# huangnengCSU/longcallR

Hardware: AMD Instinct MI355X
Metric: candidate_sites_per_sec (higher is better)
Workload: dtype u8 in, u32 counts, f64 likelihoods, i64 fixed-point phase scores

## Files before the change

longcallr_amd/csrc/k2_candidates.hip:

```cpp
#include "lcr_dev.h"
#include "k2_eval.h"

#define SCAN_ITEMS 4
#define SCAN_TILE (LCR_BLOCK * SCAN_ITEMS)

__device__ __forceinline__ int wave_incl_scan_i(int v, int lane) {
#pragma unroll
  for (int d = 1; d < 64; d <<= 1) {
    int t = __shfl_up(v, d, 64);
    if (lane >= d) v += t;
  }
  return v;
}
__device__ __forceinline__ long long wave_incl_scan_ll(long long v, int lane) {
#pragma unroll
  for (int d = 1; d < 64; d <<= 1) {
    long long t = __shfl_up(v, d, 64);
    if (lane >= d) v += t;
  }
  return v;
}

template <typename OutT>
__global__ void __launch_bounds__(LCR_BLOCK) scan_phase1(const int32_t* __restrict__ in, OutT* __restrict__ out, int32_t n,
                                                         long long* __restrict__ block_sum) {
  __shared__ long long wsum[4];
  const int tid = threadIdx.x, lane = tid & 63, w = tid >> 6;
  const long long base = (long long)blockIdx.x * SCAN_TILE + (long long)tid * SCAN_ITEMS;
  long long v[SCAN_ITEMS], s = 0;
#pragma unroll
  for (int k = 0; k < SCAN_ITEMS; k++) { v[k] = (base + k < n) ? (long long)in[base + k] : 0; s += v[k]; }
  long long incl = wave_incl_scan_ll(s, lane);
  if (lane == 63) wsum[w] = incl;
  __syncthreads();
  long long add = 0;
  for (int i = 0; i < w; i++) add += wsum[i];
  long long run = incl - s + add;
#pragma unroll
  for (int k = 0; k < SCAN_ITEMS; k++) { if (base + k < n) out[base + k] = (OutT)run; run += v[k]; }
  if (tid == LCR_BLOCK - 1) block_sum[blockIdx.x] = incl + add;
}
__global__ void __launch_bounds__(1024) scan_phase2(long long* __restrict__ block_sum, int32_t n_blocks, long long* total) {
  __shared__ long long wsum[16];
  __shared__ long long carry_s;
  const int tid = threadIdx.x, lane = tid & 63, w = tid >> 6;
  if (tid == 0) carry_s = 0;
  __syncthreads();
  for (int base = 0; base < n_blocks; base += 1024) {
    long long v = (base + tid < n_blocks) ? block_sum[base + tid] : 0;
    long long incl = wave_incl_scan_ll(v, lane);
    if (lane == 63) wsum[w] = incl;
    __syncthreads();
    long long add = carry_s;
    for (int i = 0; i < w; i++) add += wsum[i];
    if (base + tid < n_blocks) block_sum[base + tid] = incl - v + add;
    __syncthreads();
    if (tid == 1023) carry_s = incl + add;
    __syncthreads();
  }
  if (tid == 0 && total) *total = carry_s;
}
template <typename OutT>
__global__ void __launch_bounds__(LCR_BLOCK) scan_phase3(OutT* __restrict__ out, int32_t n, const long long* __restrict__ block_sum,
                                                         int write_last) {
  const long long base = (long long)blockIdx.x * SCAN_TILE + (long long)threadIdx.x * SCAN_ITEMS;
  const long long add = block_sum[blockIdx.x];
#pragma unroll
  for (int k = 0; k < SCAN_ITEMS; k++) if (base + k < n) out[base + k] += (OutT)add;
  (void)write_last;
}
#define SCAN_FUSED_BLOCKS 2048
template <typename OutT>
__global__ void __launch_bounds__(LCR_BLOCK) scan_phase3x(OutT* __restrict__ out, int32_t n, const long long* __restrict__ block_sum, int32_t n_blocks,
                                                          int32_t* __restrict__ total32, int64_t* __restrict__ total64) {
  __shared__ long long wsum[LCR_BLOCK / 64];
  const int tid = threadIdx.x, lane = tid & 63, w = tid >> 6;
  long long s = 0;
  for (int j = tid; j < (int)blockIdx.x; j += LCR_BLOCK) s += block_sum[j];
  for (int d = 32; d >= 1; d >>= 1) s += __shfl_xor(s, d, 64);
  if (lane == 0) wsum[w] = s;
  __syncthreads();
  long long add = 0;
#pragma unroll
  for (int i = 0; i < LCR_BLOCK / 64; i++) add += wsum[i];
  const long long base = (long long)blockIdx.x * SCAN_TILE + (long long)tid * SCAN_ITEMS;
#pragma unroll
  for (int k = 0; k < SCAN_ITEMS; k++) if (base + k < n) out[base + k] += (OutT)add;
  if ((int)blockIdx.x == n_blocks - 1 && tid == 0) {
    const long long tot = add + block_sum[n_blocks - 1];
    if (total32) *total32 = (int32_t)tot;
    if (total64) *total64 = (int64_t)tot;
  }
}
__global__ void write_total_i32(const long long* total, int32_t* dst) { *dst = (int32_t)*total; }
__global__ void gather_i32(const int32_t* __restrict__ src, const int32_t* __restrict__ idx, int32_t n, int32_t n_src,
                           const int32_t* __restrict__ total, int32_t* __restrict__ out, int32_t* __restrict__ host_out) {
  const int i = blockIdx.x * blockDim.x + threadIdx.x;
  if (i < n) { const int32_t v = idx[i] < n_src ? src[idx[i]] : *total; out[i] = v; if (host_out) host_out[i] = v; }
}
void launch_gather_i32(const int32_t* src, const int32_t* idx, int32_t n, int32_t n_src, const int32_t* total, int32_t* out, hipStream_t s, int32_t* host_out) {
  if (n > 0) hipLaunchKernelGGL(gather_i32, dim3((n + 255) / 256), dim3(256), 0, s, src, idx, n, n_src, total, out, host_out);
}
__global__ void write_total_i64(const long long* total, int64_t* dst) { *dst = (int64_t)*total; }

void launch_scan_i32(DevBuf& tmp, const int32_t* in, int32_t* out_excl, int32_t n, int32_t* total, hipStream_t s) {
  const int nb = (n + SCAN_TILE - 1) / SCAN_TILE;
  (void)tmp.reserve(((size_t)nb + 2) * sizeof(long long));
  long long* bs = tmp.as<long long>();
  if (n > 0 && nb <= SCAN_FUSED_BLOCKS) {
    hipLaunchKernelGGL(scan_phase1<int32_t>, dim3(nb), dim3(LCR_BLOCK), 0, s, in, out_excl, n, bs);
    hipLaunchKernelGGL(scan_phase3x<int32_t>, dim3(nb), dim3(LCR_BLOCK), 0, s, out_excl, n, bs, nb, total, (int64_t*)nullptr);
  } else if (n > 0) {
    hipLaunchKernelGGL(scan_phase1<int32_t>, dim3(nb), dim3(LCR_BLOCK), 0, s, in, out_excl, n, bs);
    hipLaunchKernelGGL(scan_phase2, dim3(1), dim3(1024), 0, s, bs, nb, bs + nb);
    hipLaunchKernelGGL(scan_phase3<int32_t>, dim3(nb), dim3(LCR_BLOCK), 0, s, out_excl, n, bs, 0);
    if (total) hipLaunchKernelGGL(write_total_i32, dim3(1), dim3(1), 0, s, bs + nb, total);
  } else if (total) {
    (void)hipMemsetAsync(total, 0, sizeof(int32_t), s);
  }
}
void launch_scan_i32_to_i64(DevBuf& tmp, const int32_t* in, int64_t* out_excl, int32_t n, hipStream_t s) {
  const int nb = (n + SCAN_TILE - 1) / SCAN_TILE;
  (void)tmp.reserve(((size_t)nb + 2) * sizeof(long long));
  long long* bs = tmp.as<long long>();
  if (n > 0 && nb <= SCAN_FUSED_BLOCKS) {
    hipLaunchKernelGGL(scan_phase1<int64_t>, dim3(nb), dim3(LCR_BLOCK), 0, s, in, out_excl, n, bs);
    hipLaunchKernelGGL(scan_phase3x<int64_t>, dim3(nb), dim3(LCR_BLOCK), 0, s, out_excl, n, bs, nb, (int32_t*)nullptr, out_excl + n);
  } else if (n > 0) {
    hipLaunchKernelGGL(scan_phase1<int64_t>, dim3(nb), dim3(LCR_BLOCK), 0, s, in, out_excl, n, bs);
    hipLaunchKernelGGL(scan_phase2, dim3(1), dim3(1024), 0, s, bs, nb, bs + nb);
    hipLaunchKernelGGL(scan_phase3<int64_t>, dim3(nb), dim3(LCR_BLOCK), 0, s, out_excl, n, bs, 0);
    hipLaunchKernelGGL(write_total_i64, dim3(1), dim3(1), 0, s, bs + nb, out_excl + n);
  } else {
    (void)hipMemsetAsync(out_excl, 0, sizeof(int64_t), s);
  }
}

__global__ void k2_sor_threshold(float* out) { *out = strand_odds_ratio(5, 5, 9, 1); }

__device__ __forceinline__ ColEval eval_column(const uint32_t* __restrict__ planes, int64_t n_cols, int64_t o, uint8_t ref_base,
                                               const DevParams& prm, const BinomTable& bt) {
  uint32_t cnt[4];
#pragma unroll
  for (int k = 0; k < 4; k++) { cnt[k] = planes[(int64_t)(LCR_PL_A + k) * n_cols + o]; }
  return eval_counts(cnt, ref_base, prm, bt,
                     [&]() { return planes[(int64_t)LCR_PL_D * n_cols + o]; }, [&]() { return planes[(int64_t)LCR_PL_N * n_cols + o]; },
                     [&](int k) { return planes[(int64_t)(LCR_PL_FWD_A + k) * n_cols + o]; });
}

__global__ void __launch_bounds__(LCR_BLOCK)
k2_filter(BatchView b, DevParams prm, BinomTable bt, const int32_t* __restrict__ tile_region, const int32_t* __restrict__ tile_col0,
          int64_t n_cols, const uint32_t* __restrict__ planes, const int32_t* __restrict__ tile_fill, uint8_t* __restrict__ flags,
          int32_t* __restrict__ tile_count) {
  __shared__ int cnt_s;
  if (tile_fill[blockIdx.x] == 0) { if (threadIdx.x == 0) tile_count[blockIdx.x] = 0; return; }
  const int g = tile_region[blockIdx.x], tc0 = tile_col0[blockIdx.x];
  const int tlen = min(LCR_TILE, b.len[g] - tc0);
  const int64_t gcol0 = b.col_off[g] + tc0;
  if (threadIdx.x == 0) cnt_s = 0;
  __syncthreads();
  int mine = 0;
  for (int col = threadIdx.x; col < tlen; col += LCR_BLOCK) {
    ColEval ev = eval_column(planes, n_cols, gcol0 + col, b.ref[gcol0 + col], prm, bt);
    flags[gcol0 + col] = ev.pass ? 1 : 0;
    mine += ev.pass ? 1 : 0;
  }
  if (mine) atomicAdd(&cnt_s, mine);
  __syncthreads();
  if (threadIdx.x == 0) tile_count[blockIdx.x] = cnt_s;
}

void launch_k2_filter(const BatchView& b, const DevParams& p, const int32_t* tile_region, const int32_t* tile_col0,
                      int32_t n_tiles, int64_t n_cols, const uint32_t* planes, const int32_t* tile_fill, uint8_t* flags,
                      int32_t* tile_count, hipStream_t s) {
  static const BinomTable bt = make_binom_table();
  if (n_tiles == 0) return;
  hipLaunchKernelGGL(k2_filter, dim3(n_tiles), dim3(LCR_BLOCK), 0, s, b, p, bt, tile_region, tile_col0, n_cols, planes,
                     tile_fill, flags, tile_count);
}

__global__ void __launch_bounds__(LCR_BLOCK)
k2_compact(BatchView b, DevParams prm, BinomTable bt, const int32_t* __restrict__ tile_region,
           const int32_t* __restrict__ tile_col0, int64_t n_cols, const uint32_t* __restrict__ planes,
           const uint8_t* __restrict__ flags, const int32_t* __restrict__ tile_count, const int32_t* __restrict__ tile_off,
           Survivor* __restrict__ out, int32_t out_cap ) {
  __shared__ int wsum[4];
  if (tile_count[blockIdx.x] == 0) return;
  const int g = tile_region[blockIdx.x], tc0 = tile_col0[blockIdx.x];
  const int tlen = min(LCR_TILE, b.len[g] - tc0);
  const int64_t gcol0 = b.col_off[g] + tc0;
  const int tid = threadIdx.x, lane = tid & 63, w = tid >> 6;
  int base = tile_off[blockIdx.x];
  int f[4], c = 0;
#pragma unroll
  for (int k = 0; k < 4; k++) { int col = tid * 4 + k; f[k] = (col < tlen) ? flags[gcol0 + col] : 0; c += f[k]; }
  int incl = wave_incl_scan_i(c, lane);
  if (lane == 63) wsum[w] = incl;
  __syncthreads();
  int add = 0;
  for (int i = 0; i < w; i++) add += wsum[i];
  int rank = base + incl - c + add;
#pragma unroll
  for (int k = 0; k < 4; k++) {
    if (!f[k]) continue;
    const int col = tid * 4 + k;
    ColEval ev = eval_column(planes, n_cols, gcol0 + col, b.ref[gcol0 + col], prm, bt);
    Survivor sv;
    sv.gcol = gcol0 + col; sv.region = g; sv.col = tc0 + col;
    sv.ref_base = ev.ref_base; sv.allele1 = ev.allele1; sv.allele2 = ev.allele2; sv.n_alt = ev.n_alt;
    sv.cnt1 = ev.cnt1; sv.cnt2 = ev.cnt2; sv.depth = ev.depth; sv.af1 = ev.af1; sv.af2 = ev.af2;
    sv.ts_fwd = planes[(int64_t)LCR_PL_TS_FWD * n_cols + gcol0 + col];
    sv.ts_rev = planes[(int64_t)LCR_PL_TS_REV * n_cols + gcol0 + col];
    if (rank < out_cap) out[rank] = sv;
    rank++;
  }
}


__global__ void __launch_bounds__(LCR_BLOCK)
k2_hist(BatchView b, DevParams prm, const ReadBin* __restrict__ rbin, const Survivor* __restrict__ sv,
        const int32_t* __restrict__ tile_off, int32_t n_tiles, int32_t n_sv, uint32_t* __restrict__ hist, int32_t* __restrict__ hit_cnt, uint2* __restrict__ hit_list,
        int32_t* __restrict__ ovf_cnt, int32_t* __restrict__ ovf_list) {
  const int r = (blockIdx.x * LCR_BLOCK + threadIdx.x) >> 4;
  const bool live = r < b.n_reads;
  const int rr = live ? r : 0;
  const ReadBin h = rbin[rr];
  const int rend = b.read_rend[rr];
  const uint8_t* __restrict__ seq = b.bases + h.seq_off;
  const uint8_t* __restrict__ qual = b.quals + h.seq_off;
  const int l16 = threadIdx.x & 15, rbase = threadIdx.x & 48;
  const int key = h.rel_pos > 0 ? h.rel_pos : 0, rend_c = min(rend, h.vec);
  const bool span = live && rend_c > key;
  const int t0 = h.ftile + (int)((unsigned int)key / (unsigned int)LCR_TILE), t1 = h.ftile + (int)((unsigned int)(max(rend_c, 1) - 1) / (unsigned int)LCR_TILE) + 1;
  uint32_t pre[4];
  {
    const uint32_t* __restrict__ cg = b.cigar + h.cig_off;
#pragma unroll
    for (int k = 0; k < 4; k++) pre[k] = (span && (uint32_t)(16 * k + l16) < (uint32_t)h.n_cig) ? cg[16 * k + l16] : 0u;
  }
  const int s_lo = span ? tile_off[t0] : 0, s_hi = span ? (t1 < n_tiles ? tile_off[t1] : n_sv) : 0;
  int nh = 0;
  uint2* const hl = hit_cnt ? hit_list + (size_t)rr * LCR_HITS : nullptr;
  int cur, s_end;
  auto site_col = [&](int i) { return sv[i].col; };
  row16_find_sites(span && s_lo < s_hi, h, rend, s_lo, s_hi, site_col, &cur, &s_end);
  row16_walk_range(b, h, cur, s_end, pre, site_col,
    [&](int cur_s, int c, bool hit) {
      uint8_t base = 0, rq = 0;
      if (hit) { base = seq[c]; rq = qual[c]; }
      if (hl) {
        const unsigned int hm = (unsigned int)(__ballot(hit) >> rbase) & 0xffffu;
        const int at = nh + __popc(hm & ((1u << l16) - 1u));
        if (hit && at < LCR_HITS) hl[at] = make_uint2((uint32_t)cur_s, (uint32_t)base | ((uint32_t)rq << 8));
        nh += __popc(hm);
      }
      if (!hit) return;
      const uint8_t bq = rq < 30 ? rq : 30;
      bool masked = false;
      if (in_end_zone(c, h.lead, h.reb, prm.dist_to_end))
        masked = prm.ont ? true : polya_masked(seq, b.seq_len[rr], c, prm.polya_len, sv[cur_s].ref_base);
      const int bi = base_code(base);
      if (!masked && bi >= 0) atomicAdd(&hist[((int64_t)cur_s * 4 + bi) * 31 + bq], 1u);
    });
  if (hl && live && l16 == 0) {
    hit_cnt[r] = nh;
    if (nh > LCR_HITS) ovf_list[atomicAdd(ovf_cnt, 1)] = r;
  }
}

void launch_k2_hist(const BatchView& b, const DevParams& p, const ReadBin* rbin, const Survivor* sv,
                    const int32_t* tile_off, int32_t n_tiles, int32_t n_sv, uint32_t* hist, int32_t* hit_cnt, void* hit_list, int32_t* ovf_cnt, int32_t* ovf_list, hipStream_t s) {
  if (b.n_reads == 0) return;
  const int per = LCR_BLOCK / 16;
  hipLaunchKernelGGL(k2_hist, dim3((b.n_reads + per - 1) / per), dim3(LCR_BLOCK), 0, s, b, p, rbin, sv, tile_off, n_tiles, n_sv, hist, hit_cnt, (uint2*)hit_list,
                     ovf_cnt, ovf_list);
}

#ifndef HT_SLOTS
#define HT_SLOTS 256
#endif
#ifndef HT_SPLIT
#define HT_SPLIT 32
#endif
#ifndef HT_BLOCK
#define HT_BLOCK 512
#endif
__global__ void __launch_bounds__(HT_BLOCK)
k2_hist_tiles(BatchView b, const int32_t* __restrict__ tile_col0, const int32_t* __restrict__ tile_count, const int32_t* __restrict__ tile_off,
              const Survivor* __restrict__ sv, const int32_t* __restrict__ ent_off, const uint2* __restrict__ ents,
              const unsigned long long* __restrict__ recs, uint32_t* __restrict__ hist) {
  const int tile = blockIdx.x / HT_SPLIT, part = blockIdx.x % HT_SPLIT, cnt = tile_count[tile];
  if (cnt == 0) return;
  __shared__ uint32_t hp[HT_SLOTS * 62];
  __shared__ uint16_t slot_of[LCR_TILE];
  constexpr int HT_LANES = 8;
  const int tid = threadIdx.x, grp = tid / HT_LANES, ln = tid % HT_LANES;
  const int s0 = tile_off[tile], tc0 = tile_col0[tile];
  const int e0 = ent_off[tile];
  const int n_ent = ent_off[tile + 1] - e0;
  const int j_lo = 16 * (int)((int64_t)n_ent * part / HT_SPLIT), j_hi = 16 * (int)((int64_t)n_ent * (part + 1) / HT_SPLIT);
  if (j_lo >= j_hi) return;
  for (int p0 = 0; p0 < cnt; p0 += HT_SLOTS) {
    const int pc = min(HT_SLOTS, cnt - p0);
    for (int i = tid; i < LCR_TILE; i += HT_BLOCK) slot_of[i] = 0xFFFFu;
    for (int i = tid; i < pc * 62; i += HT_BLOCK) hp[i] = 0u;
    __syncthreads();
    for (int i = tid; i < pc; i += HT_BLOCK) slot_of[sv[s0 + p0 + i].col - tc0] = (uint16_t)i;
    __syncthreads();
    const int c_lo = sv[s0 + p0].col - tc0, c_hi = sv[s0 + p0 + pc - 1].col - tc0;
    auto fetch = [&](int j) -> unsigned long long {
      if (j >= j_hi) return ~0ull;
      const uint2 en = ents[e0 + (j >> 4)];
      return ((unsigned int)j & 15u) < en.y ? recs[en.x + ((unsigned int)j & 15u)] : ~0ull;
    };
    unsigned long long nx = fetch(j_lo + grp), nx2 = fetch(j_lo + grp + HT_BLOCK / HT_LANES);
    for (int j = j_lo + grp; j < j_hi; j += HT_BLOCK / HT_LANES) {
      const unsigned long long rec = nx;
      nx = nx2;
      nx2 = fetch(j + 2 * (HT_BLOCK / HT_LANES));
      const unsigned long long off = rec & REC_OFF_MASK;
      const bool live = off < REC_KIND_N;
      const int col0 = (int)((rec >> 40) & 1023u), len = (int)((rec >> 50) & 1023u) + 1;
      const int d_lo = max(0, c_lo - col0), d_hi = live ? min(len - 1, c_hi - col0) : -1;
      auto tally = [&](int dd, bool in, uint32_t base, uint32_t qual) {
        const uint32_t slot = slot_of[min(col0 + max(dd, 0), LCR_TILE - 1)];
        const uint32_t u = (base & 0xDFu) - 65u;
        const bool acgt = u < 20u && ((0x80045u >> u) & 1u);
        const uint32_t k = ((base & 0xDFu) >> 1) & 3u, bi = k ^ (k >> 1);
        const uint32_t q = min(qual, 30u);
        const uint32_t idx = slot * 124u + bi * 31u + q;
        if (in && acgt && slot != 0xFFFFu) atomicAdd(&hp[idx >> 1], 1u << (16 * (idx & 1u)));
      };
      for (int d0 = d_lo + 4 * ln; d0 <= d_hi; d0 += 4 * HT_LANES) {
        const unsigned long long at = off + (unsigned long long)d0;
        uint32_t bw, qw;
        if (at + 4 <= (unsigned long long)b.n_bases) {
          bw = *reinterpret_cast<const uint32_t*>(b.bases + at); qw = *reinterpret_cast<const uint32_t*>(b.quals + at);
        } else {
          bw = 0; qw = 0;
          for (int t = 0; t < 4; t++) if (at + t < (unsigned long long)b.n_bases) { bw |= (uint32_t)b.bases[at + t] << (8 * t); qw |= (uint32_t)b.quals[at + t] << (8 * t); }
        }
#pragma unroll
        for (int t = 0; t < 4; t++) tally(d0 + t, d0 + t <= d_hi, (bw >> (8 * t)) & 0xFFu, (qw >> (8 * t)) & 0xFFu);
      }
    }
    __syncthreads();
    uint32_t* out = hist + (int64_t)(s0 + p0) * 124;
    for (int i = tid; i < pc * 124; i += HT_BLOCK) {
      const uint32_t v = (hp[i >> 1] >> (16 * (i & 1))) & 0xffffu;
      if (v) atomicAdd(&out[i], v);
    }
    __syncthreads();
  }
}

void launch_k2_hist_tiles(const BatchView& b, const int32_t* tile_col0, int32_t n_tiles, const int32_t* tile_count,
                          const int32_t* tile_off, const Survivor* sv, const int32_t* ent_off, const void* ents, const unsigned long long* recs,
                          uint32_t* hist , hipStream_t s) {
  if (n_tiles == 0) return;
  hipLaunchKernelGGL(k2_hist_tiles, dim3((unsigned)n_tiles * HT_SPLIT), dim3(HT_BLOCK), 0, s, b, tile_col0, tile_count, tile_off, sv, ent_off,
                     (const uint2*)ents, recs, hist);
}

struct GtConst {
  double le[31], l1e[31];
  double log10_2;
  double log_prior[3];
};
static GtConst make_gt_const() {
  GtConst c;
  for (int q = 0; q <= 30; q++) {
    double e = pow(0.1, (double)q / 10.0);
    c.le[q] = log10(e);
    c.l1e[q] = log10(1.0 - e);
  }
  c.log10_2 = log10(2.0);
  const double theta = 0.001;
  c.log_prior[0] = log10(theta / 2.0); c.log_prior[1] = log10(theta); c.log_prior[2] = log10(1.0 - 1.5 * theta);
  return c;
}

__global__ void __launch_bounds__(LCR_BLOCK)
k2_gt(DevParams prm, GtConst gc, const Survivor* __restrict__ sv, int32_t n_sv, const uint32_t* __restrict__ hist,
      const int64_t* __restrict__ start0, lcr_candidate* __restrict__ out, int32_t* __restrict__ keep) {
  const int s = blockIdx.x * blockDim.x + threadIdx.x;
  if (s >= n_sv) return;
  const Survivor v = sv[s];
  const uint32_t* h = hist + (int64_t)s * 124;
  keep[s] = 0;
  const int ri = base_code(v.ref_base);
  {
    int ai = -1; uint32_t ac = 0;
    if (v.allele1 != v.ref_base) { ai = base_code(v.allele1); ac = v.cnt1; }
    else if (v.allele2 != v.ref_base) { ai = base_code(v.allele2); ac = v.cnt2; }
    if (ai >= 0) {
      uint32_t pass = 0;
      for (uint32_t q = prm.min_baseq; q <= 30; q++) pass += h[ai * 31 + q];
      if (ac > 0 && pass < 2) return;
    }
  }
  double l0 = 0.0, l2 = 0.0;
  uint32_t num_reads = 0;
  for (int q = 0; q <= 30; q++) {
    const uint32_t hm = h[ri * 31 + q];
    uint32_t hx = 0;
#pragma unroll
    for (int bq = 0; bq < 4; bq++) if (bq != ri) hx += h[bq * 31 + q];
    num_reads += hm + hx;
    if (hm) { l0 += (double)hm * gc.le[q]; l2 += (double)hm * gc.l1e[q]; }
    if (hx) { l0 += (double)hx * gc.l1e[q]; l2 += (double)hx * gc.le[q]; }
  }
  double loglik[3] = {l0, 0.0, l2};
  loglik[1] -= (double)num_reads * gc.log10_2;
  double logprob[3] = {loglik[0] + gc.log_prior[0], loglik[1] + gc.log_prior[1], loglik[2] + gc.log_prior[2]};
  const double mlp = fmax(fmax(logprob[0], logprob[1]), logprob[2]);
  double vp[3] = {pow(10.0, logprob[0] - mlp), pow(10.0, logprob[1] - mlp), pow(10.0, logprob[2] - mlp)};
  const double svp = vp[0] + vp[1] + vp[2];
  vp[2] = vp[2] / svp;
  const double variant_quality = -10.0 * log10(fmax(10e-301, vp[2]));
  const double ml = fmax(fmax(loglik[0], loglik[1]), loglik[2]);
  double gl[3] = {pow(10.0, loglik[0] - ml), pow(10.0, loglik[1] - ml), pow(10.0, loglik[2] - ml)};
  const double sgl = gl[0] + gl[1] + gl[2];
  double gp[3] = {gl[0] / sgl, gl[1] / sgl, gl[2] / sgl};
  double ph[3] = {-10.0 * log10(gp[0]), -10.0 * log10(gp[1]), -10.0 * log10(gp[2])};
  for (int i = 1; i < 3; i++) {
    double x = ph[i];
    int j = i;
    while (j > 0 && x < ph[j - 1]) { ph[j] = ph[j - 1]; j--; }
    ph[j] = x;
  }
  const double genotype_quality = ph[1] - ph[0];

  lcr_candidate c;
  c.pos = start0[v.region] + v.col;
  c.region = v.region;
  c.ref_base = v.ref_base; c.allele1 = v.allele1; c.allele2 = v.allele2; c.n_alt = v.n_alt;
  c.cnt1 = v.cnt1; c.cnt2 = v.cnt2; c.depth = v.depth; c.af1 = v.af1; c.af2 = v.af2;
  c.haplotype = 0; c.phase_set = 0; c.phase_score = 0.0;
  for (int k = 0; k < 3; k++) { c.loglik[k] = loglik[k]; c.gt_prob[k] = gp[k]; }
  c.qual = variant_quality; c.gq = genotype_quality;
  if (gp[0] > gp[1] && gp[0] > gp[2]) { c.variant_type = 2; c.genotype = -1; }
  else if (gp[1] > gp[0] && gp[1] > gp[2]) { c.variant_type = 1; c.genotype = 0; }
  else { c.variant_type = 0; c.genotype = 1; }
  c.flags = 0;
  if (variant_quality < (double)prm.min_qual) return;
  uint8_t ref_allele_base, alt0; float altf0, altf1 = 0.0f;
  if (v.allele1 == v.ref_base) { ref_allele_base = v.allele1; alt0 = v.allele2; altf0 = v.af2; }
  else if (v.allele2 == v.ref_base) { ref_allele_base = v.allele2; alt0 = v.allele1; altf0 = v.af1; }
  else { ref_allele_base = v.ref_base; alt0 = v.allele1; altf0 = v.af1; altf1 = v.af2; }
  const int fwd_t = (int)v.ts_fwd, rev_t = (int)v.ts_rev;
  bool kept = false;
  if (ref_allele_base == 'A' && alt0 == 'G' && (fwd_t > rev_t * 2 || (fwd_t == 0 && rev_t == 0)) && c.variant_type != 2) {
    c.flags = LCR_F_RNA_EDIT; kept = true;
  } else if (ref_allele_base == 'T' && alt0 == 'C' && (rev_t > fwd_t * 2 || (fwd_t == 0 && rev_t == 0)) && c.variant_type != 2) {
    c.flags = LCR_F_RNA_EDIT; kept = true;
  } else if (v.n_alt == 1 && altf0 < prm.min_af) {
    c.flags = LCR_F_CAND_SOMATIC; kept = true;
  } else if (c.variant_type == 2) {
    if (v.n_alt == 2 && altf0 >= prm.min_af && altf1 >= prm.min_af) { c.variant_type = 3; c.genotype = -1; }
    c.flags = LCR_F_HOM | LCR_F_FOR_PHASING; kept = true;
  } else if (c.variant_type == 1) {
    if (v.n_alt == 2) { c.variant_type = 3; c.genotype = -1; c.flags = LCR_F_HOM | LCR_F_FOR_PHASING; }
    else c.flags = LCR_F_HET | LCR_F_FOR_PHASING;
    kept = true;
  }
  if (!kept) return;
  out[s] = c;
  keep[s] = 1;
}

void launch_k2_gt(const DevParams& p, const Survivor* sv, int32_t n_sv, const uint32_t* hist, const int64_t* start0,
                  lcr_candidate* out, int32_t* keep, hipStream_t s) {
  static const GtConst g_gtc = make_gt_const();
  if (n_sv == 0) return;
  hipLaunchKernelGGL(k2_gt, dim3((n_sv + LCR_BLOCK - 1) / LCR_BLOCK), dim3(LCR_BLOCK), 0, s, p, g_gtc, sv, n_sv, hist, start0, out, keep);
}

void launch_k2_compact(const BatchView& b, const DevParams& p, const int32_t* tile_region, const int32_t* tile_col0,
                       int32_t n_tiles, int64_t n_cols, const uint32_t* planes, const uint8_t* flags,
                       const int32_t* tile_count, const int32_t* tile_off, Survivor* out, int32_t out_cap, hipStream_t s) {
  static const BinomTable bt = make_binom_table();
  if (n_tiles == 0) return;
  hipLaunchKernelGGL(k2_compact, dim3(n_tiles), dim3(LCR_BLOCK), 0, s, b, p, bt, tile_region, tile_col0, n_cols,
                     planes, flags, tile_count, tile_off, out, out_cap);
}

float lcr_device_sor_threshold(hipStream_t s) {
  float* d = nullptr;
  float h = 0.f;
  if (hipMalloc(&d, sizeof(float)) != hipSuccess) return 0.f;
  hipLaunchKernelGGL(k2_sor_threshold, dim3(1), dim3(1), 0, s, d);
  (void)hipMemcpyAsync(&h, d, sizeof(float), hipMemcpyDeviceToHost, s);
  (void)hipStreamSynchronize(s);
  (void)hipFree(d);
  return h;
}

__global__ void __launch_bounds__(LCR_BLOCK)
k2_scatter(const lcr_candidate* __restrict__ tmp, const int32_t* __restrict__ keep, const int32_t* __restrict__ pos, int32_t n_sv,
           lcr_candidate* __restrict__ out, const int32_t* __restrict__ sv_region_off, int32_t n_regions, int32_t* __restrict__ cand_off) {
  const int64_t id = (int64_t)blockIdx.x * LCR_BLOCK + threadIdx.x;
  if (id <= n_regions) cand_off[id] = sv_region_off[id] < n_sv ? pos[sv_region_off[id]] : pos[n_sv];
  const int s = (int)(id >> 3), w = (int)(id & 7);
  if (s >= n_sv || !keep[s]) return;
  reinterpret_cast<uint4*>(out + pos[s])[w] = reinterpret_cast<const uint4*>(tmp + s)[w];
}
__global__ void __launch_bounds__(256)
k2_dense(lcr_candidate* __restrict__ cand, const int32_t* __restrict__ cand_off, int32_t n_regions, int32_t* __restrict__ idx,
         uint32_t dense_win, uint32_t min_dense_cnt, lcr_candidate* __restrict__ h_cand, int32_t* __restrict__ h_off) {
  __shared__ int wcnt[4], base_s;
  const int g = blockIdx.x, tid = threadIdx.x, lane = tid & 63, w = tid >> 6;
  const int lo = cand_off[g], hi = cand_off[g + 1];
  int32_t* concat = idx + lo;
  if (tid == 0) base_s = 0;
  __syncthreads();
  for (int i0 = lo; i0 < hi; i0 += 256) {
    const int i = i0 + tid;
    const bool keep = i < hi && (cand[i].flags & (LCR_F_HOM | LCR_F_HET)) != 0;
    const unsigned long long m = __ballot(keep);
    if (lane == 0) wcnt[w] = __popcll(m);
    __syncthreads();
    int before = base_s;
    for (int k = 0; k < w; k++) before += wcnt[k];
    if (keep) concat[before + __popcll(m & ((1ull << lane) - 1ull))] = i;
    __syncthreads();
    if (tid == 0) base_s += wcnt[0] + wcnt[1] + wcnt[2] + wcnt[3];
    __syncthreads();
  }
  const int n = base_s;
  auto mark = [&](int i, int j) {
    for (int tk = i; tk < j; tk++) { atomicOr(&cand[concat[tk]].flags, (uint32_t)LCR_F_DENSE); atomicAnd(&cand[concat[tk]].flags, ~(uint32_t)LCR_F_FOR_PHASING); }
  };
  auto sweep = [&](int i, int64_t W, uint32_t cnt) {
    const int64_t start_pos = cand[concat[i]].pos;
    int j = i;
    while (j < n && cand[concat[j]].pos - start_pos <= W) j++;
    if (j < n) { if ((uint32_t)(j - i) >= cnt) mark(i, j); }
    else if ((uint32_t)(n - i) >= cnt) mark(i, n - 1);
  };
  for (int i = tid; i < n; i += 256) {
    sweep(i, (int64_t)dense_win, min_dense_cnt);
    sweep(i, 4, 3u);
  }
  if (!h_cand) return;
  __syncthreads();
  const uint4* src = reinterpret_cast<const uint4*>(cand + lo);
  uint4* dst = reinterpret_cast<uint4*>(h_cand + lo);
  const int n16 = (hi - lo) * (int)(sizeof(lcr_candidate) / 16);
  for (int i = tid; i < n16; i += 256) dst[i] = src[i];
  if (tid == 0) { h_off[g] = lo; if (g == n_regions - 1) h_off[n_regions] = hi; }
}
void launch_k2_finish(DevBuf& scan_tmp, const lcr_candidate* tmp, const int32_t* keep, int32_t n_sv, const int32_t* sv_region_off,
                      int32_t n_regions, int32_t* pos , int32_t* idx , lcr_candidate* out,
                      int32_t* cand_off , uint32_t dense_win, uint32_t min_dense_cnt, hipStream_t s,
                      lcr_candidate* h_cand , int32_t* h_off ) {
  static_assert(sizeof(lcr_candidate) % 16 == 0, "k2_dense exports 16-byte words");
  launch_scan_i32(scan_tmp, keep, pos, n_sv, pos + n_sv, s);
  if (n_sv > 0) {
    const int64_t nthreads = std::max<int64_t>((int64_t)n_sv * 8, (int64_t)n_regions + 1);
    hipLaunchKernelGGL(k2_scatter, dim3((unsigned)((nthreads + LCR_BLOCK - 1) / LCR_BLOCK)), dim3(LCR_BLOCK), 0, s, tmp, keep, pos, n_sv, out,
                       sv_region_off, n_regions, cand_off);
  } else launch_gather_i32(pos, sv_region_off, n_regions + 1, n_sv, pos + n_sv, cand_off, s);
  if (n_regions > 0) hipLaunchKernelGGL(k2_dense, dim3(n_regions), dim3(256), 0, s, out, cand_off, n_regions, idx, dense_win, min_dense_cnt, h_cand, h_off);
}
```

longcallr_amd/csrc/lcr_api.hip:

```cpp
#include <atomic>
#include <thread>
#include <algorithm>
#include <cmath>
#include <cstring>
#include <cstdlib>

#include <chrono>
#include "lcr_dev.h"
#include "lcr_phase_host.h"

struct lcr_ctx {
  int device = 0;
  hipStream_t stream = nullptr;
  bool own_stream = false;
  std::string err;

  bool loaded = false;
  BatchView bv{};
  int64_t n_cols = 0, n_bases = 0, n_cigar = 0;
  int32_t n_tiles = 0;
  std::vector<int64_t> h_start0, h_col_off;
  std::vector<int32_t> h_len, h_read_begin, h_region_first_tile;
  DevBuf in_[16];
  struct UploadSlot { DevBuf buf[16]; hipEvent_t ev = nullptr; bool filled = false; lcr_reads rd{}; lcr_regions rg{}; } up[2];
  hipStream_t up_stream = nullptr;
  hipEvent_t ev_dl = nullptr, ev_cand_dl = nullptr;
  bool cand_dl_other = false;
  int bound_slot = -1;
  bool bound_host = false;
  DevBuf scan_tmp, read_region, read_bin, read_rend, tile_region, tile_col0, first_tile, k0_tile_fill, k0_items, tile_nbase, tile_order;
  DevBuf desc_tile, desc_val, chunks, chunk_off;
  DevBuf blk_first_read, read_scan, cig_compact, cig_off_new, cig_new_off32;
  uint64_t cig0 = 0;
  uint32_t n_ops = 0;
  int64_t n_items = 0;

  bool have_planes = false;
  DevBuf planes;
  DevParams dp{};
  int32_t pile_platform = -1; uint32_t pile_dist_to_end = 0;
  float sor_thr = -1.f;
  HostBuf h_planes;
  HostBuf h_nnz;
  DevBuf region_e_off, frag_tmp_col, frag_tmp_val;
  hipEvent_t ev_nnz = nullptr, ev_cand = nullptr, ev_ctl = nullptr, ev_sv = nullptr;
  int32_t sv_cap_guess = 0;
  bool nnz_pending = false, cand_pending = false;
  HostBuf h_order;
  static constexpr int UP_LANES = 4;
  HostBuf h_up[2 * UP_LANES]; hipEvent_t ev_up[2 * UP_LANES] = {}; bool up_busy[2 * UP_LANES] = {};
  HostBuf h_stage[4];

  bool have_cand = false;
  bool cand_used = false;
  DevBuf flags, tile_count, tile_off, total, survivors, sv_region_off, hist, cand_tmp, keep;
  DevBuf hit_cnt, hit_list, ovf_list;
  bool hits_valid = false; int32_t hits_n_sv = 0;
  int dbg_hist_tiles = 0;
  int dbg_spec_compact = 1;
  int dbg_fuse_filter = 1;
  bool flt_fused = false;
  DevParams flt_dp{};
  int dbg_k3_hits = 1;
  std::vector<lcr_candidate> h_cand;
  std::vector<int32_t> h_cand_off;
  DevBuf d_cand, d_cand_off;
  DevBuf imp_pos, imp_gt, imp_q, imp_cnt;
  HostBuf h_imp_bad;
  hipEvent_t ev_imp = nullptr;

  bool have_frag = false;
  uint32_t min_linkers = 1;
  int32_t n_rows = 0;
  int64_t nnz = 0;
  std::vector<int32_t> h_row_region_off;
  DevBuf region_rows, row_region_off, row_cnt, row_links, row_ptr, col, val;
  HostBuf h_row_ptr, h_row_read, h_col, h_val, h_row_fp, h_row_links;

  bool have_phase = false;
  bool res_valid = false;
  int32_t res_ng = 0;
  int phase_slot = -1;
  PhaseHost phase;
  std::vector<int32_t> ld_off, ld_snps;

  DevBuf rd_start, rd_end, rd_diff, rd_ex, rd_cnt, rd_off, rd_s, rd_e, rd_max;
  std::vector<int64_t> rl_start0;
  std::vector<int32_t> rl_len;
  std::vector<uint32_t> rl_max;

  bool timing = false;
  uint32_t timing_mask = 0;
  hipEvent_t ev[LCR_NKERNELS][2] = {};
  bool ev_valid[LCR_NKERNELS] = {};
  int64_t pileup_bytes = 0, stage_bytes = 0;
};

#include <map>
#include <mutex>
namespace {
struct BlockCache {
  std::mutex mu;
  std::multimap<size_t, void*> blocks[2][16];
  size_t held[2][16] = {};
  size_t limit[2] = {(size_t)24 << 30, (size_t)2 << 30};
};
BlockCache& block_cache() { static BlockCache* c = new BlockCache(); return *c; }
}
void* lcr_cache_take(int host, size_t want, size_t* cap) {
  int dev = 0;
  if (hipGetDevice(&dev) != hipSuccess || dev < 0 || dev >= 16) return nullptr;
  BlockCache& bc = block_cache();
  std::lock_guard<std::mutex> g(bc.mu);
  auto& m = bc.blocks[host ? 1 : 0][dev];
  auto it = m.lower_bound(want);
  if (it == m.end() || it->first > 2 * want + (1u << 20)) return nullptr;
  void* p = it->second;
  *cap = it->first;
  bc.held[host ? 1 : 0][dev] -= it->first;
  m.erase(it);
  return p;
}
bool lcr_cache_put(int host, void* p, size_t cap) {
  int dev = 0;
  if (!p || hipGetDevice(&dev) != hipSuccess || dev < 0 || dev >= 16) return false;
  BlockCache& bc = block_cache();
  std::lock_guard<std::mutex> g(bc.mu);
  const int h = host ? 1 : 0;
  if (bc.held[h][dev] + cap > bc.limit[h]) return false;
  bc.blocks[h][dev].emplace(cap, p);
  bc.held[h][dev] += cap;
  return true;
}

namespace {

struct Timer {
  lcr_ctx* c; int k;
  bool on() const { return c->timing && (c->timing_mask == 0 || ((c->timing_mask >> k) & 1u)); }
  Timer(lcr_ctx* c_, int k_) : c(c_), k(k_) { if (on()) { (void)hipEventRecord(c->ev[k][0], c->stream); } }
  ~Timer() { if (on()) { (void)hipEventRecord(c->ev[k][1], c->stream); c->ev_valid[k] = true; } }
};

DevParams to_dev(const lcr_params* p, float sor_thr) {
  DevParams d{};
  d.ont = p->platform == LCR_PLATFORM_ONT;
  d.dist_to_end = (int32_t)p->dist_to_end;
  d.polya_len = (int32_t)p->polya_len;
  d.min_baseq = p->min_baseq; d.min_depth = p->min_depth; d.max_depth = p->max_depth; d.min_qual = p->min_qual;
  d.low_cnt_cut = p->low_cnt_cut; d.min_linkers = p->min_linkers; d.use_strand_bias = p->use_strand_bias;
  d.min_af = p->min_af; d.min_af_intron = p->min_af_intron; d.low_frac_cut = p->low_frac_cut;
  d.sor_threshold = sor_thr;
  return d;
}

int upload_bytes(lcr_ctx* c, void* dst, const void* src, size_t bytes, hipStream_t q = nullptr) {
  if (!q) q = c->stream;
  if (bytes <= 64 * 1024) { HIPCHK(c, hipMemcpyAsync(dst, src, bytes, hipMemcpyHostToDevice, q)); return LCR_OK; }
  hipPointerAttribute_t at{};
  if (hipPointerGetAttributes(&at, src) == hipSuccess && at.type == hipMemoryTypeHost) {
    HIPCHK(c, hipMemcpyAsync(dst, src, bytes, hipMemcpyHostToDevice, q));
    return LCR_OK;
  }
  (void)hipGetLastError();
  constexpr size_t CH = 8u << 20;
  const int lanes = bytes >= (64u << 20) ? lcr_ctx::UP_LANES : 1;
  for (int k = 0; k < 2 * lanes; k++) {
    HIPCHK(c, c->h_up[k].reserve(CH));
    if (!c->ev_up[k]) HIPCHK(c, hipEventCreateWithFlags(&c->ev_up[k], hipEventDisableTiming));
  }
  const size_t n_ch = (bytes + CH - 1) / CH;
  std::atomic<int> bad{0};
  auto lane_fn = [&](int w) {
    (void)hipSetDevice(c->device);
    int use = 0;
    for (size_t i = (size_t)w; i < n_ch && !bad.load(std::memory_order_relaxed); i += (size_t)lanes, use ^= 1) {
      const int k = 2 * w + use;
      const size_t off = i * CH, n = std::min(CH, bytes - off);
      hipError_t e = c->up_busy[k] ? hipEventSynchronize(c->ev_up[k]) : hipSuccess;
      if (e == hipSuccess) {
        memcpy(c->h_up[k].p, (const uint8_t*)src + off, n);
        e = hipMemcpyAsync((uint8_t*)dst + off, c->h_up[k].p, n, hipMemcpyHostToDevice, q);
      }
      if (e == hipSuccess) e = hipEventRecord(c->ev_up[k], q);
      if (e != hipSuccess) { bad.store((int)e); return; }
      c->up_busy[k] = true;
    }
  };
  if (lanes == 1) lane_fn(0);
  else {
    std::vector<std::thread> th;
    try { for (int w = 1; w < lanes; w++) th.emplace_back(lane_fn, w); } catch (...) { }
    const int started = (int)th.size() + 1;
    lane_fn(0);
    for (auto& t : th) t.join();
    for (int w = started; w < lanes; w++) lane_fn(w);
  }
  if (bad.load()) { c->err = std::string("host upload: ") + hipGetErrorString((hipError_t)bad.load()); return LCR_E_DEVICE; }
  return LCR_OK;
}

template <class T>
int upload(lcr_ctx* c, DevBuf& buf, const T* src, size_t n, const T** dst, int mem) {
  if (mem == LCR_MEM_DEVICE) { *dst = src; return LCR_OK; }
  HIPCHK(c, buf.reserve(std::max<size_t>(n, 1) * sizeof(T)));
  if (n) { const int rc = upload_bytes(c, buf.p, src, n * sizeof(T)); if (rc) return rc; }
  *dst = buf.as<T>();
  return LCR_OK;
}

}

int g_lcr_own_fill = 1;
namespace {
__global__ void __launch_bounds__(256) lcr_fill_kernel(uint8_t* p, uint32_t word, size_t head, size_t n16, size_t tail) {
  const size_t t = (size_t)blockIdx.x * blockDim.x + threadIdx.x, nt = (size_t)gridDim.x * blockDim.x;
  if (t < head) p[t] = (uint8_t)word;
  uint4* const body = reinterpret_cast<uint4*>(p + head);
  const uint4 w = make_uint4(word, word, word, word);
  for (size_t i = t; i < n16; i += nt) body[i] = w;
  if (t < tail) p[head + 16 * n16 + t] = (uint8_t)word;
}
}
namespace {
struct FillRanges { uint8_t* p[4]; size_t head[4], n16[4], tail[4]; uint32_t word[4]; };
__global__ void __launch_bounds__(256) lcr_fill_multi_kernel(FillRanges r) {
  const int k = blockIdx.y;
  uint8_t* const p = r.p[k];
  if (!p) return;
  const size_t t = (size_t)blockIdx.x * blockDim.x + threadIdx.x, nt = (size_t)gridDim.x * blockDim.x;
  const uint32_t word = r.word[k];
  if (t < r.head[k]) p[t] = (uint8_t)word;
  uint4* const body = reinterpret_cast<uint4*>(p + r.head[k]);
  const uint4 w = make_uint4(word, word, word, word);
  for (size_t i = t; i < r.n16[k]; i += nt) body[i] = w;
  if (t < r.tail[k]) p[r.head[k] + 16 * r.n16[k] + t] = (uint8_t)word;
}
}
hipError_t lcr_fill_multi_async(int n, void* const* ptrs, const int* bytes_val, const size_t* sizes, hipStream_t s) {
  if (!g_lcr_own_fill) { for (int k = 0; k < n; k++) if (sizes[k]) { const hipError_t e = hipMemsetAsync(ptrs[k], bytes_val[k], sizes[k], s); if (e != hipSuccess) return e; } return hipSuccess; }
  FillRanges r{};
  size_t most = 0;
  int m = 0;
  for (int k = 0; k < n && m < 4; k++) {
    if (!sizes[k]) continue;
    const size_t mis = (size_t)((uintptr_t)ptrs[k] & 15), head = std::min(sizes[k], mis ? 16 - mis : 0), n16 = (sizes[k] - head) / 16;
    const uint32_t b = (uint32_t)(bytes_val[k] & 255);
    r.p[m] = (uint8_t*)ptrs[k]; r.head[m] = head; r.n16[m] = n16; r.tail[m] = sizes[k] - head - 16 * n16; r.word[m] = b | (b << 8) | (b << 16) | (b << 24);
    most = std::max(most, n16); m++;
  }
  if (!m) return hipSuccess;
  const unsigned blocks = (unsigned)std::max<size_t>(1, std::min<size_t>((most + 255) / 256, 1024));
  hipLaunchKernelGGL(lcr_fill_multi_kernel, dim3(blocks, (unsigned)m), dim3(256), 0, s, r);
  return hipGetLastError();
}

hipError_t lcr_fill_async(void* p, int byte, size_t bytes, hipStream_t s) {
  if (!bytes) return hipSuccess;
  if (!g_lcr_own_fill) return hipMemsetAsync(p, byte, bytes, s);
  const size_t mis = (size_t)((uintptr_t)p & 15), head = std::min(bytes, mis ? 16 - mis : 0), n16 = (bytes - head) / 16, tail = bytes - head - 16 * n16;
  const uint32_t b = (uint32_t)(byte & 255), word = b | (b << 8) | (b << 16) | (b << 24);
  const unsigned blocks = (unsigned)std::max<size_t>(1, std::min<size_t>((n16 + 255) / 256, 2048));
  hipLaunchKernelGGL(lcr_fill_kernel, dim3(blocks), dim3(256), 0, s, (uint8_t*)p, word, head, n16, tail);
  return hipGetLastError();
}

int g_lcr_host_trace = 0;
namespace {
struct HtMark { const char* tag; std::chrono::steady_clock::time_point t; };
thread_local std::vector<HtMark> g_ht;
}
void lcr_host_trace_mark(const char* tag) { g_ht.push_back({tag, std::chrono::steady_clock::now()}); }
void lcr_host_trace_flush() {
  if (g_ht.empty()) return;
  std::string line = "[host]";
  char buf[96];
  for (const HtMark& m : g_ht) { snprintf(buf, sizeof buf, " %s %.1f", m.tag, std::chrono::duration<double, std::micro>(m.t - g_ht[0].t).count()); line += buf; }
  fprintf(stderr, "%s\n", line.c_str());
  g_ht.clear();
}

extern "C" {

const char* lcr_version(void) { return "liblcr 0.1 (gfx950)"; }

int lcr_release_cached_memory(void) {
  BlockCache& bc = block_cache();
  std::lock_guard<std::mutex> g(bc.mu);
  int cur = 0;
  (void)hipGetDevice(&cur);
  for (int dev = 0; dev < 16; dev++) {
    if (bc.blocks[0][dev].empty() && bc.blocks[1][dev].empty()) continue;
    (void)hipSetDevice(dev);
    for (auto& kv : bc.blocks[0][dev]) (void)hipFree(kv.second);
    for (auto& kv : bc.blocks[1][dev]) (void)hipHostFree(kv.second);
    bc.blocks[0][dev].clear(); bc.blocks[1][dev].clear();
    bc.held[0][dev] = bc.held[1][dev] = 0;
  }
  (void)hipSetDevice(cur);
  return LCR_OK;
}
int lcr_set_cache_limits(int64_t device_bytes, int64_t host_bytes) {
  if (device_bytes < 0 || host_bytes < 0) return LCR_E_ARG;
  BlockCache& bc = block_cache();
  std::lock_guard<std::mutex> g(bc.mu);
  bc.limit[0] = (size_t)device_bytes; bc.limit[1] = (size_t)host_bytes;
  return LCR_OK;
}

int lcr_params_preset(int preset, lcr_params* o) {
  if (!o || preset < 0 || preset > 3) return LCR_E_ARG;
  memset(o, 0, sizeof *o);
  const bool ont = preset >= 2;
  o->platform = ont ? LCR_PLATFORM_ONT : LCR_PLATFORM_HIFI;
  o->min_baseq = 10; o->dist_to_end = ont ? 20 : 40; o->polya_len = 5;
  o->min_depth = ont ? 10 : 6; o->max_depth = 50000; o->min_qual = 2;
  o->dense_win = 100; o->min_dense_cnt = 5; o->low_cnt_cut = 10; o->min_linkers = 1; o->max_enum_snps = 10;
  o->ld_weight_threshold = 1;
  o->use_strand_bias = (preset == 0 || preset == 2) ? 1 : 0;
  o->min_af = ont ? 0.20f : 0.15f; o->min_af_intron = 0.0f; o->low_frac_cut = 0.05f;
  o->min_phase_score = ont ? 13.0f : 11.0f;
  o->read_assign_cutoff = 0.0; o->seed = 2025;
  return LCR_OK;
}

int lcr_ctx_create(int device, lcr_ctx** out) {
  if (!out) return LCR_E_ARG;
  int n = 0;
  if (hipGetDeviceCount(&n) != hipSuccess || n <= 0 || device < 0 || device >= n) return LCR_E_DEVICE;
  if (hipSetDevice(device) != hipSuccess) return LCR_E_DEVICE;
  lcr_ctx* c = new lcr_ctx();
  c->device = device;
  if (hipStreamCreateWithFlags(&c->stream, hipStreamNonBlocking) != hipSuccess) { delete c; return LCR_E_DEVICE; }
  c->own_stream = true;
  for (int k = 0; k < LCR_NKERNELS; k++)
    for (int j = 0; j < 2; j++)
      if (hipEventCreate(&c->ev[k][j]) != hipSuccess) { delete c; return LCR_E_DEVICE; }
  *out = c;
  return LCR_OK;
}

void lcr_ctx_destroy(lcr_ctx* c) {
  if (!c) return;
  (void)hipSetDevice(c->device);
  if (c->cand_pending && c->cand_dl_other && c->ev_cand_dl) (void)hipEventSynchronize(c->ev_cand_dl);
  (void)c->phase.settle(nullptr);
  for (hipStream_t q : {c->phase.main_q, c->phase.side, c->phase.aux}) if (q) (void)hipStreamSynchronize(q);
  (void)hipStreamSynchronize(c->stream);
  if (c->up_stream) (void)hipStreamSynchronize(c->up_stream);
  for (auto& u : c->up) if (u.ev) (void)hipEventDestroy(u.ev);
  if (c->up_stream) (void)hipStreamDestroy(c->up_stream);
  for (hipEvent_t e : {c->ev_dl, c->ev_cand_dl, c->ev_nnz, c->ev_cand, c->ev_sv, c->ev_ctl, c->ev_imp}) if (e) (void)hipEventDestroy(e);
  for (int k = 0; k < 2 * lcr_ctx::UP_LANES; k++) if (c->ev_up[k]) (void)hipEventDestroy(c->ev_up[k]);
  c->phase.release();
  for (int k = 0; k < LCR_NKERNELS; k++) for (int j = 0; j < 2; j++) if (c->ev[k][j]) (void)hipEventDestroy(c->ev[k][j]);
  if (c->own_stream && c->stream) (void)hipStreamDestroy(c->stream);
  delete c;
}

const char* lcr_last_error(const lcr_ctx* c) { return c ? c->err.c_str() : "null ctx"; }

static int phase_settle(lcr_ctx* c) { return c->phase.settle(&c->err); }

int lcr_ctx_set_stream(lcr_ctx* c, void* s) {
  if (!c) return LCR_E_ARG;
  (void)hipSetDevice(c->device);
  { int rc = phase_settle(c); if (rc) return rc; }
  if (c->own_stream && c->stream) { (void)hipStreamSynchronize(c->stream); (void)hipStreamDestroy(c->stream); }
  if (s) { c->stream = (hipStream_t)s; c->own_stream = false; }
  else { HIPCHK(c, hipStreamCreateWithFlags(&c->stream, hipStreamNonBlocking)); c->own_stream = true; }
  return LCR_OK;
}

int lcr_ctx_sync(lcr_ctx* c) {
  if (!c) return LCR_E_ARG;
  HIPCHK(c, hipSetDevice(c->device));
  { int rc = phase_settle(c); if (rc) return rc; }
  if (c->cand_pending && c->cand_dl_other) HIPCHK(c, hipEventSynchronize(c->ev_cand_dl));
  HIPCHK(c, hipStreamSynchronize(c->stream));
  return LCR_OK;
}

int lcr_enable_timing(lcr_ctx* c, int on) { if (!c) return LCR_E_ARG; c->timing = on != 0; return LCR_OK; }

int lcr_kernel_ms(lcr_ctx* c, int k, float* ms) {
  if (!c || !ms || k < 0 || k >= LCR_NKERNELS) return LCR_E_ARG;
  if (!c->ev_valid[k]) return LCR_E_STATE;
  HIPCHK(c, hipEventSynchronize(c->ev[k][1]));
  HIPCHK(c, hipEventElapsedTime(ms, c->ev[k][0], c->ev[k][1]));
  return LCR_OK;
}

int lcr_pileup_bytes(lcr_ctx* c, int64_t* bytes) {
  if (!c || !bytes) return LCR_E_ARG;
  *bytes = c->pileup_bytes;
  return LCR_OK;
}

int lcr_pileup_stage_bytes(lcr_ctx* c, int64_t* bytes) {
  if (!c || !bytes) return LCR_E_ARG;
  *bytes = c->stage_bytes;
  return LCR_OK;
}

int lcr_load_batch(lcr_ctx* c, const lcr_reads* rd, const lcr_regions* rg) {
  if (!c || !rd || !rg) return LCR_E_ARG;
  if (rd->n_reads < 0 || rg->n_regions < 0 || rd->mem != rg->mem) { c->err = "bad batch header"; return LCR_E_ARG; }
  HIPCHK(c, hipSetDevice(c->device));
  if (rd->mem == LCR_MEM_HOST) { int rc = phase_settle(c); if (rc) return rc; }
  c->loaded = c->have_planes = c->have_cand = c->have_frag = c->have_phase = c->cand_used = false;
  c->bound_slot = -1;
  c->bound_host = rd->mem == LCR_MEM_HOST;
  const int nr = rd->n_reads, ng = rg->n_regions, mem = rd->mem;
  c->h_start0.assign(ng, 0); c->h_len.assign(ng, 0); c->h_col_off.assign(ng + 1, 0); c->h_read_begin.assign(ng + 1, 0);
  if (mem == LCR_MEM_HOST) {
    if (ng) { memcpy(c->h_start0.data(), rg->start0, ng * sizeof(int64_t)); memcpy(c->h_len.data(), rg->len, ng * sizeof(int32_t)); }
    memcpy(c->h_col_off.data(), rg->col_off, (ng + 1) * sizeof(int64_t));
    memcpy(c->h_read_begin.data(), rg->read_begin, (ng + 1) * sizeof(int32_t));
  } else {
    const size_t o1 = (size_t)ng * 8, o2 = o1 + (size_t)(ng + 1) * 8, o3 = o2 + (size_t)ng * 4, tot = o3 + (size_t)(ng + 1) * 4;
    HIPCHK(c, c->h_stage[0].reserve(tot + 16));
    HIPCHK(c, c->first_tile.reserve((ng + 1) * 4));
    uint8_t* st = c->h_stage[0].as<uint8_t>();
    uint8_t* dst = nullptr;
    HIPCHK(c, hipHostGetDevicePointer((void**)&dst, st, 0));
    HIPCHK(c, c->h_order.reserve(64));
    memset(c->h_order.p, 0, 64);
    { int32_t* d_flag = nullptr; HIPCHK(c, hipHostGetDevicePointer((void**)&d_flag, c->h_order.p, 0));
      Timer t(c, LCR_K_BIND_TABLE);
      launch_k0_bind_a(rg->start0, rg->len, rg->col_off, rg->read_begin, ng, c->first_tile.as<int32_t>(), (int64_t*)dst,
                       (int32_t*)(dst + o2), (int64_t*)(dst + o1), (int32_t*)(dst + o3), rd->cig_off, rd->n_cig, nr, rd->n_cigar, d_flag, c->stream); }
    HIPCHK(c, hipStreamSynchronize(c->stream));
    HIPCHK(c, hipGetLastError());
    if (ng) { memcpy(c->h_start0.data(), st, ng * sizeof(int64_t)); memcpy(c->h_len.data(), st + o2, ng * sizeof(int32_t)); }
    memcpy(c->h_col_off.data(), st + o1, (ng + 1) * sizeof(int64_t));
    memcpy(c->h_read_begin.data(), st + o3, (ng + 1) * sizeof(int32_t));
  }
  if (c->h_read_begin[ng] != nr || c->h_col_off[0] != 0) { c->err = "read_begin/col_off inconsistent"; return LCR_E_ARG; }
  for (int g = 0; g < ng; g++)
    if (c->h_len[g] < 0 || c->h_col_off[g + 1] - c->h_col_off[g] != c->h_len[g] || c->h_read_begin[g + 1] < c->h_read_begin[g]) {
      c->err = "region table inconsistent"; return LCR_E_ARG;
    }
  c->n_cols = c->h_col_off[ng];
  if (c->n_cols + ng + 1 > (int64_t)INT32_MAX) { c->err = "batch too large: columns + regions must stay below 2^31; split it"; return LCR_E_ARG; }
  c->n_bases = rd->n_bases; c->n_cigar = rd->n_cigar;

  BatchView& b = c->bv;
  b.n_reads = nr; b.n_regions = ng; b.n_bases = rd->n_bases;
  int rc;
#define UP(i, field, T, n) if ((rc = upload<T>(c, c->in_[i], (const T*)rd->field, (size_t)(n), (const T**)&b.field, mem))) return rc
  UP(0, pos, int32_t, nr); UP(1, seq_len, int32_t, nr);
  if ((rc = upload<int32_t>(c, c->in_[2], rd->lead_clip, nr, &b.lead, mem))) return rc;
  if ((rc = upload<int32_t>(c, c->in_[3], rd->trail_clip, nr, &b.trail, mem))) return rc;
  UP(4, flags, uint8_t, nr); UP(5, seq_off, uint64_t, nr); UP(6, cig_off, uint64_t, nr); UP(7, n_cig, uint32_t, nr);
  UP(8, bases, uint8_t, rd->n_bases); UP(9, quals, uint8_t, rd->n_bases); UP(10, cigar, uint32_t, rd->n_cigar);
#undef UP
  if ((rc = upload<int64_t>(c, c->in_[11], rg->start0, ng, &b.start0, mem))) return rc;
  if ((rc = upload<int32_t>(c, c->in_[12], rg->len, ng, &b.len, mem))) return rc;
  if ((rc = upload<int64_t>(c, c->in_[13], rg->col_off, ng + 1, &b.col_off, mem))) return rc;
  if ((rc = upload<int32_t>(c, c->in_[14], rg->read_begin, ng + 1, &b.read_begin, mem))) return rc;
  if ((rc = upload<uint8_t>(c, c->in_[15], rg->ref, c->n_cols, &b.ref, mem))) return rc;

  c->h_region_first_tile.assign(ng + 1, 0);
  for (int g = 0; g < ng; g++) c->h_region_first_tile[g + 1] = c->h_region_first_tile[g] + (c->h_len[g] + LCR_TILE - 1) / LCR_TILE;
  c->n_tiles = c->h_region_first_tile[ng];
  HIPCHK(c, c->tile_region.reserve(std::max<size_t>(c->n_tiles, 1) * 4));
  HIPCHK(c, c->tile_col0.reserve(std::max<size_t>(c->n_tiles, 1) * 4));
  HIPCHK(c, c->first_tile.reserve((ng + 1) * 4));
  if (mem == LCR_MEM_HOST)
    launch_k0_region_setup(b.start0, b.len, b.col_off, b.read_begin, ng, c->first_tile.as<int32_t>(), nullptr, nullptr, nullptr, nullptr, c->stream);
  HIPCHK(c, c->read_rend.reserve(std::max<size_t>(nr, 1) * 4));
  b.read_rend = c->read_rend.as<int32_t>();
  HIPCHK(c, c->read_region.reserve(std::max(nr, 1) * 4));
  b.read_region = c->read_region.as<int32_t>();
  b.region_first_tile = c->first_tile.as<int32_t>(); b.error_flag = nullptr;
  HIPCHK(c, c->read_bin.reserve(std::max<size_t>(nr, 1) * sizeof(ReadBin)));
  bool contiguous = true, cig_oob = false;
  uint64_t cig0 = 0, cig_end = 0, cig_total = 0;
  if (mem == LCR_MEM_HOST) {
    HIPCHK(c, c->h_order.reserve(64));
    HIPCHK(c, hipStreamSynchronize(c->stream));
    memset(c->h_order.p, 0, 64);
    if (nr) { cig0 = rd->cig_off[0]; cig_end = rd->cig_off[nr - 1] + rd->n_cig[nr - 1]; }
    for (int r = 0; r + 1 < nr && contiguous; r++) contiguous = rd->cig_off[r + 1] == rd->cig_off[r] + rd->n_cig[r];
    for (int r = 0; r < nr; r++) {
      cig_total += rd->n_cig[r];
      cig_oob |= rd->cig_off[r] > (uint64_t)rd->n_cigar || (uint64_t)rd->n_cig[r] > (uint64_t)rd->n_cigar - rd->cig_off[r];
    }
  } else {
    const uint64_t* g = reinterpret_cast<const uint64_t*>(c->h_order.as<uint8_t>() + 16);
    contiguous = c->h_order.as<int32_t>()[1] == 0;
    cig_oob = c->h_order.as<int32_t>()[2] != 0;
    cig0 = g[0]; cig_end = g[1];
  }
  if (cig_oob) { c->err = "cig_off / n_cig reach beyond n_cigar"; return LCR_E_ARG; }
  if (!contiguous && (rd->n_cigar > 0x7FFFFFF0ll || cig_total > 0x7FFFFFF0ull)) { c->err = "batch too large: CIGAR ops must stay below 2^31; split it"; return LCR_E_ARG; }
  if (!contiguous) {
    HIPCHK(c, c->cig_new_off32.reserve(((size_t)nr + 2) * 4));
    HIPCHK(c, c->cig_off_new.reserve(std::max<size_t>(nr, 1) * 8));
    int32_t* total = c->cig_new_off32.as<int32_t>() + nr;
    launch_scan_i32(c->scan_tmp, (const int32_t*)b.n_cig, c->cig_new_off32.as<int32_t>(), nr, total, c->stream);
    int32_t h_total = 0;
    HIPCHK(c, hipMemcpyAsync(&h_total, total, 4, hipMemcpyDeviceToHost, c->stream));
    HIPCHK(c, hipStreamSynchronize(c->stream));
    if (h_total < 0) { c->err = "batch too large: CIGAR ops must stay below 2^31; split it"; return LCR_E_ARG; }
    HIPCHK(c, c->cig_compact.reserve(std::max<size_t>((size_t)h_total, 1) * 4));
    launch_k0_cig_compact(b.cigar, b.cig_off, b.n_cig, c->cig_new_off32.as<int32_t>(), nr, c->cig_compact.as<uint32_t>(),
                          c->cig_off_new.as<uint64_t>(), c->stream);
    b.cigar = c->cig_compact.as<uint32_t>(); b.cig_off = c->cig_off_new.as<uint64_t>();
    cig0 = 0; cig_end = (uint64_t)h_total;
  }
  if (cig_end < cig0 || cig_end - cig0 > 0xFFF00000ull || (contiguous && cig_end > (uint64_t)std::max<int64_t>(rd->n_cigar, 0))) {
    c->err = "cig_off / n_cig inconsistent with n_cigar, or more than 2^32 CIGAR ops in one batch"; return LCR_E_ARG;
  }
  c->cig0 = cig0; c->n_ops = (uint32_t)(cig_end - cig0);
  *c->h_order.as<int32_t>() = 0;
  { int32_t* d_flag = nullptr; HIPCHK(c, hipHostGetDevicePointer((void**)&d_flag, c->h_order.p, 0));
    const int opb = launch_k0_opb();
    const int32_t n_blocks = (int32_t)(((uint64_t)c->n_ops + opb - 1) / opb);
    HIPCHK(c, c->blk_first_read.reserve(((size_t)n_blocks + 2) * 4));
    Timer t(c, LCR_K_BIND);
    launch_k0_bind_b(b, c->read_bin.as<ReadBin>(), d_flag, c->read_region.as<int32_t>(), c->n_tiles, c->tile_region.as<int32_t>(), c->tile_col0.as<int32_t>(),
                     c->cig0, opb, n_blocks, c->blk_first_read.as<int32_t>(), c->stream); }
  if (mem == LCR_MEM_HOST) HIPCHK(c, hipStreamSynchronize(c->stream));
  HIPCHK(c, hipGetLastError());
  c->loaded = true;
  return LCR_OK;
}

int lcr_load_batch_async(lcr_ctx* c, const lcr_reads* rd, const lcr_regions* rg, int32_t slot) {
  if (!c || !rd || !rg) return LCR_E_ARG;
  if (slot < 0 || slot > 1) { c->err = "lcr_load_batch_async: slot must be 0 or 1"; return LCR_E_ARG; }
  if (rd->mem != LCR_MEM_HOST || rg->mem != LCR_MEM_HOST) { c->err = "lcr_load_batch_async takes LCR_MEM_HOST batches (a device-resident batch needs no upload)"; return LCR_E_ARG; }
  if (rd->n_reads < 0 || rg->n_regions < 0 || rd->n_bases < 0 || rd->n_cigar < 0) { c->err = "bad batch header"; return LCR_E_ARG; }
  HIPCHK(c, hipSetDevice(c->device));
  if (c->phase.pending && c->phase_slot == slot) { int rc = phase_settle(c); if (rc) return rc; }
  if (!c->up_stream) HIPCHK(c, hipStreamCreateWithFlags(&c->up_stream, hipStreamNonBlocking));
  lcr_ctx::UploadSlot& u = c->up[slot];
  if (!u.ev) HIPCHK(c, hipEventCreateWithFlags(&u.ev, hipEventDisableTiming));
  if (c->bound_slot == slot) {
    HIPCHK(c, hipStreamSynchronize(c->stream));
    c->loaded = c->have_planes = c->have_cand = c->have_frag = c->have_phase = c->cand_used = false;
    c->bound_slot = -1;
  }
  u.filled = false;
  const int nr = rd->n_reads, ng = rg->n_regions;
  int64_t n_cols = 0;
  if (ng) { if (!rg->col_off) { c->err = "col_off missing"; return LCR_E_ARG; } n_cols = rg->col_off[ng]; }
  if (n_cols < 0) { c->err = "region table inconsistent"; return LCR_E_ARG; }
  u.rd = lcr_reads{}; u.rg = lcr_regions{};
  u.rd.mem = LCR_MEM_DEVICE; u.rg.mem = LCR_MEM_DEVICE;
  u.rd.n_reads = nr; u.rd.n_bases = rd->n_bases; u.rd.n_cigar = rd->n_cigar; u.rg.n_regions = ng;
  auto put = [&](int i, const void* src, size_t bytes, const void** dst) -> int {
    HIPCHK(c, u.buf[i].reserve(std::max<size_t>(bytes, 1)));
    if (bytes) {
      if (!src) { c->err = "lcr_load_batch_async: null array"; return LCR_E_ARG; }
      { const int rc2 = upload_bytes(c, u.buf[i].p, src, bytes, c->up_stream); if (rc2) return rc2; }
    }
    *dst = u.buf[i].p;
    return LCR_OK;
  };
  int rc;
#define PUT(i, obj, field, T, n) if ((rc = put(i, (obj)->field, (size_t)(n) * sizeof(T), (const void**)&u.obj.field))) return rc
  PUT(0, rd, pos, int32_t, nr); PUT(1, rd, seq_len, int32_t, nr); PUT(2, rd, lead_clip, int32_t, nr); PUT(3, rd, trail_clip, int32_t, nr);
  PUT(4, rd, flags, uint8_t, nr); PUT(5, rd, seq_off, uint64_t, nr); PUT(6, rd, cig_off, uint64_t, nr); PUT(7, rd, n_cig, uint32_t, nr);
  PUT(8, rd, bases, uint8_t, rd->n_bases); PUT(9, rd, quals, uint8_t, rd->n_bases); PUT(10, rd, cigar, uint32_t, rd->n_cigar);
  PUT(11, rg, start0, int64_t, ng); PUT(12, rg, len, int32_t, ng); PUT(13, rg, col_off, int64_t, ng + 1); PUT(14, rg, read_begin, int32_t, ng + 1);
  PUT(15, rg, ref, uint8_t, n_cols);
#undef PUT
  HIPCHK(c, hipEventRecord(u.ev, c->up_stream));
  u.filled = true;
  return LCR_OK;
}

int lcr_bind_batch(lcr_ctx* c, int32_t slot) {
  if (!c) return LCR_E_ARG;
  if (slot < 0 || slot > 1) { c->err = "lcr_bind_batch: slot must be 0 or 1"; return LCR_E_ARG; }
  lcr_ctx::UploadSlot& u = c->up[slot];
  if (!u.filled) { c->err = "lcr_bind_batch before lcr_load_batch_async on this slot"; return LCR_E_STATE; }
  HIPCHK(c, hipSetDevice(c->device));
  HIPCHK(c, hipStreamWaitEvent(c->stream, u.ev, 0));
  const int rc = lcr_load_batch(c, &u.rd, &u.rg);
  if (rc == LCR_OK) c->bound_slot = slot;
  return rc;
}

int lcr_host_alloc(size_t bytes, void** out) {
  if (!out) return LCR_E_ARG;
  *out = nullptr;
  return hipHostMalloc(out, std::max<size_t>(bytes, 1), hipHostMallocDefault) == hipSuccess ? LCR_OK : LCR_E_NOMEM;
}
void lcr_host_free(void* p) { if (p) (void)hipHostFree(p); }
int lcr_host_register(void* p, size_t bytes) {
  if (!p || !bytes) return LCR_E_ARG;
  return hipHostRegister(p, bytes, hipHostRegisterDefault) == hipSuccess ? LCR_OK : LCR_E_DEVICE;
}
int lcr_host_unregister(void* p) { return p && hipHostUnregister(p) == hipSuccess ? LCR_OK : LCR_E_ARG; }

int lcr_pileup(lcr_ctx* c, const lcr_params* p) {
  HT("pileup");
  if (!c || !p) return LCR_E_ARG;
  if (!c->loaded) { c->err = "lcr_pileup before lcr_load_batch"; return LCR_E_STATE; }
  if (p->polya_len == 0) { c->err = "polya_len must be >= 1"; return LCR_E_ARG; }
  if ((uint64_t)c->bv.n_reads * 2ull * p->dist_to_end > 0x7FFFFF00ull * (uint64_t)LCR_BLOCK) { c->err = "dist_to_end x reads too large for one launch; split the batch"; return LCR_E_ARG; }
  HIPCHK(c, hipSetDevice(c->device));
  if (c->sor_thr < 0.f) c->sor_thr = lcr_device_sor_threshold(c->stream);
  c->dp = to_dev(p, c->sor_thr);
  c->dp.dbg = 0;
  HIPCHK(c, c->planes.reserve(std::max<size_t>((size_t)c->n_cols * LCR_NPLANES, 1) * 4));
  bool gated = false;
  BatchView& b = c->bv;
  const int nt = c->n_tiles;
  const int opb = launch_k0_opb();
  const int32_t n_blocks = (int32_t)(((uint64_t)c->n_ops + opb - 1) / opb);
  size_t desc_cap64 = (size_t)n_blocks * 128 + (size_t)b.n_reads / 4 + 1024;
  size_t pool_cap64 = (size_t)c->n_ops + (size_t)c->n_ops / 2 + (size_t)b.n_reads + (size_t)c->n_bases / LCR_TILE + 8 * desc_cap64 + 1024;
  const size_t o_ndiff = (size_t)nt + 16, o_nch = o_ndiff + nt + 8, o_cur = o_nch + nt + 8, o_acct = o_cur + nt + 8;
  const size_t o_tmp = o_acct + launch_k0_acct_words();
  const size_t fill_words = (o_tmp + launch_k1_tiles_tmp_words(nt) + 63) & ~(size_t)63;
  HIPCHK(c, c->k0_tile_fill.reserve(fill_words * 4));
  int32_t* const fill = c->k0_tile_fill.as<int32_t>();
  b.error_flag = fill + nt + 4;
  HIPCHK(c, c->tile_order.reserve(std::max(nt, 1) * 4));
  HIPCHK(c, c->tile_nbase.reserve(std::max(nt, 1) * 4));
  HIPCHK(c, c->chunk_off.reserve(((size_t)nt + 2) * 4));
  HIPCHK(c, c->read_scan.reserve(std::max<size_t>(b.n_reads, 1) * 8));
  HIPCHK(c, c->h_stage[0].reserve(64));
  int32_t n_recs = 0, bad = 0, n_ops = 0;
  const bool fuse = c->dbg_fuse_filter != 0 && c->dp.ont && nt > 0;
  c->flt_fused = false;
  if (fuse) { HIPCHK(c, c->flags.reserve(std::max<size_t>(c->n_cols, 1))); HIPCHK(c, c->tile_count.reserve(std::max(nt, 1) * 4)); }
  for (;;) {
    const size_t nsh = (size_t)launch_k0_acct_slots();
    const size_t pool_sub64 = (pool_cap64 + nsh - 1) / nsh + 256, desc_sub64 = (desc_cap64 + nsh - 1) / nsh + 64;
    if (pool_sub64 * nsh > 0xFFFFFFF0ull || desc_sub64 * nsh > 0x7FFFFFF0ull) { c->err = "batch too large for the 32-bit record pool: split it"; return LCR_E_ARG; }
    const unsigned int pool_sub = (unsigned int)pool_sub64, desc_sub = (unsigned int)desc_sub64;
    HIPCHK(c, c->k0_items.reserve(pool_sub64 * nsh * 8));
    HIPCHK(c, c->desc_tile.reserve(desc_sub64 * nsh * 4));
    HIPCHK(c, c->desc_val.reserve(desc_sub64 * nsh * 8));
    HIPCHK(c, c->chunks.reserve((pool_sub64 * nsh / 16 + desc_sub64 * nsh + 16) * 8));
    HIPCHK(c, lcr_fill_async(fill, 0, fill_words * 4, c->stream));
    if (!gated) { HIPCHK(c, c->phase.gate_stream(c->stream)); gated = true; }
    { Timer t(c, LCR_K_SPANS);
      launch_k0_ops(b, c->read_bin.as<ReadBin>(), c->blk_first_read.as<int32_t>(), c->cig0, c->n_ops, c->dp.ont, c->dp.dist_to_end, nt,
                    fill, fill + o_nch, fill + o_ndiff, fill + nt + 1, (unsigned int*)(fill + o_acct), pool_sub, c->k0_items.as<unsigned long long>(),
                    desc_sub, c->desc_tile.as<uint32_t>(), c->desc_val.p, c->read_scan.p, c->stream); }
    int32_t* const ctl = c->h_stage[0].as<int32_t>();
    if (!c->ev_ctl) HIPCHK(c, hipEventCreateWithFlags(&c->ev_ctl, hipEventDisableTiming));
    { Timer t(c, LCR_K_PILEUP);
      if (nt > 0) {
        unsigned int* d_ctl = nullptr;
        HIPCHK(c, hipHostGetDevicePointer((void**)&d_ctl, ctl, 0));
        launch_k1_tiles_a(nt, fill, fill + o_ndiff, fill + o_nch, fill + o_tmp, (unsigned int*)(fill + o_acct), launch_k0_acct_slots(),
                          (unsigned int*)(fill + nt + 1), d_ctl, c->stream);
      } else HIPCHK(c, hipMemcpyAsync(ctl, fill + nt + 1, 32, hipMemcpyDeviceToHost, c->stream));
      HIPCHK(c, hipEventRecord(c->ev_ctl, c->stream));
      if (nt > 0) launch_k1_tiles_b(nt, fill, fill + o_ndiff, fill + o_nch, fill + o_tmp, c->tile_nbase.as<int32_t>(), c->chunk_off.as<int32_t>(),
                                    c->tile_order.as<int32_t>(), c->stream);
      if (nt > 0 && c->n_ops > 0)
        launch_k0_desc_bin(fill + nt + 1, (const unsigned int*)(fill + o_acct), desc_sub, c->desc_tile.as<uint32_t>(), c->desc_val.p, c->chunk_off.as<int32_t>(), fill + o_cur,
                           c->chunks.p, n_blocks / 8 + 1, c->stream);
      launch_k1_pileup(b, c->dp, c->tile_region.as<int32_t>(), c->tile_col0.as<int32_t>(), nt, c->n_cols, fill, c->chunk_off.as<int32_t>(),
                       c->chunks.p, c->k0_items.as<unsigned long long>(), c->tile_nbase.as<int32_t>(), c->planes.as<uint32_t>(),
                       c->tile_order.as<int32_t>(), fill + o_tmp, c->stream, fuse ? c->flags.as<uint8_t>() : nullptr, fuse ? c->tile_count.as<int32_t>() : nullptr);
      if (!c->dp.ont && c->dp.dist_to_end > 0)
        launch_k1_zonefix(b, c->read_bin.as<ReadBin>(), c->dp.dist_to_end, c->dp.polya_len, c->n_cols, c->planes.as<uint32_t>(), c->stream); }
    HIPCHK(c, hipGetLastError());
    HIPCHK(c, hipEventSynchronize(c->ev_ctl));
  HT("pile:ctl");
    n_ops = ctl[1]; n_recs = ctl[2]; bad = ctl[3];
    if (*c->h_order.as<int32_t>() != 0) { c->err = "the reads of a region must be sorted by position (lcr_reads.pos)"; return LCR_E_ARG; }
    if (bad == 1) { c->err = "unknown CIGAR operation (reference panics: util.rs:944)"; return LCR_E_CIGAR; }
    if (bad == 2) { c->err = "CIGAR inconsistent with l_seq / soft clips"; return LCR_E_CIGAR; }
    if (bad == 0) break;
    pool_cap64 = std::max<size_t>(pool_cap64 * 2, ((size_t)(uint32_t)ctl[0] + 1024) * nsh);
    desc_cap64 = std::max<size_t>(desc_cap64 * 2, ((size_t)(uint32_t)ctl[4] + 1024) * nsh);
  }
  c->n_items = n_recs;
  c->pileup_bytes = c->n_bases + 8 * (int64_t)n_ops + (4 * LCR_NPLANES + 1) * c->n_cols;
  c->stage_bytes = c->n_bases + 4 * c->n_cigar + 37 * (int64_t)b.n_reads + (4 * LCR_NPLANES + 1) * c->n_cols;
  c->have_planes = true;
  c->have_cand = c->have_frag = c->have_phase = c->cand_used = false;
  c->flt_fused = fuse; c->flt_dp = c->dp;
  c->pile_platform = p->platform; c->pile_dist_to_end = p->dist_to_end;
  return LCR_OK;
}

int lcr_get_columns(lcr_ctx* c, lcr_columns* out) {
  if (!c || !out) return LCR_E_ARG;
  if (!c->have_planes) { c->err = "lcr_get_columns before lcr_pileup"; return LCR_E_STATE; }
  const size_t bytes = (size_t)c->n_cols * LCR_NPLANES * 4;
  HIPCHK(c, c->h_planes.reserve(std::max<size_t>(bytes, 1)));
  if (bytes) HIPCHK(c, hipMemcpyAsync(c->h_planes.p, c->planes.p, bytes, hipMemcpyDeviceToHost, c->stream));
  HIPCHK(c, hipStreamSynchronize(c->stream));
  out->n_cols = c->n_cols;
  out->planes = c->h_planes.as<uint32_t>();
  return LCR_OK;
}

static int cand_settle(lcr_ctx* c);
static int read_records_fresh(lcr_ctx* c);

int lcr_candidates(lcr_ctx* c, const lcr_params* p) {
  HT("cand");
  if (!c || !p) return LCR_E_ARG;
  if (!c->have_planes) { c->err = "lcr_candidates before lcr_pileup"; return LCR_E_STATE; }
  if (p->platform != c->pile_platform || p->dist_to_end != c->pile_dist_to_end) {
    c->err = "lcr_candidates: platform and dist_to_end must be those of lcr_pileup";
    return LCR_E_ARG;
  }
  HIPCHK(c, hipSetDevice(c->device));
  { int rc = phase_settle(c); if (rc) return rc; }
  HT("cand:settled");
  c->res_valid = false;
  c->dp = to_dev(p, c->dp.sor_threshold);
  const int ng = c->bv.n_regions, nt = c->n_tiles;
  if (c->cand_pending && c->cand_dl_other) HIPCHK(c, hipEventSynchronize(c->ev_cand_dl));
  HIPCHK(c, c->flags.reserve(std::max<size_t>(c->n_cols, 1)));
  HIPCHK(c, c->tile_count.reserve(std::max(nt, 1) * 4));
  HIPCHK(c, c->tile_off.reserve((std::max(nt, 1) + 1) * 4));
  HIPCHK(c, c->total.reserve(16));
  const DevParams &fa = c->flt_dp, &fb = c->dp;
  const bool have_flt = c->flt_fused && c->dbg_fuse_filter != 0 && fa.ont == fb.ont && fa.min_depth == fb.min_depth && fa.max_depth == fb.max_depth && fa.low_cnt_cut == fb.low_cnt_cut &&
                        fa.use_strand_bias == fb.use_strand_bias && fa.min_af_intron == fb.min_af_intron && fa.low_frac_cut == fb.low_frac_cut && fa.sor_threshold == fb.sor_threshold;
  { Timer t(c, LCR_K_CAND_FILTER);
    if (!have_flt) {
      c->flt_fused = false;
      launch_k2_filter(c->bv, c->dp, c->tile_region.as<int32_t>(), c->tile_col0.as<int32_t>(), nt, c->n_cols,
                       c->planes.as<uint32_t>(), c->k0_tile_fill.as<int32_t>(), c->flags.as<uint8_t>(), c->tile_count.as<int32_t>(), c->stream);
    }
  }
  HIPCHK(c, c->sv_region_off.reserve((ng + 1) * 4));
  HIPCHK(c, c->h_stage[0].reserve((ng + 2) * 4));
  int32_t* const sv_off = c->h_stage[0].as<int32_t>();
  { int32_t* d_sv = nullptr;
    HIPCHK(c, hipHostGetDevicePointer((void**)&d_sv, sv_off, 0));
    launch_scan_i32(c->scan_tmp, c->tile_count.as<int32_t>(), c->tile_off.as<int32_t>(), nt, c->total.as<int32_t>(), c->stream);
    launch_gather_i32(c->tile_off.as<int32_t>(), c->first_tile.as<int32_t>(), ng + 1, nt, c->total.as<int32_t>(), c->sv_region_off.as<int32_t>(), c->stream, d_sv); }
  const int32_t cap_guess = (c->dbg_spec_compact && nt > 0) ? c->sv_cap_guess : 0;
  if (cap_guess > 0) {
    if (!c->ev_sv) HIPCHK(c, hipEventCreateWithFlags(&c->ev_sv, hipEventDisableTiming));
    HIPCHK(c, hipEventRecord(c->ev_sv, c->stream));
    HIPCHK(c, c->survivors.reserve((size_t)cap_guess * sizeof(Survivor)));
    HIPCHK(c, c->hist.reserve((size_t)cap_guess * 124 * 4 + 64));
    HIPCHK(c, lcr_fill_async(c->hist.p, 0, (size_t)cap_guess * 124 * 4 + 64, c->stream));
    launch_k2_compact(c->bv, c->dp, c->tile_region.as<int32_t>(), c->tile_col0.as<int32_t>(), nt, c->n_cols,
                      c->planes.as<uint32_t>(), c->flags.as<uint8_t>(), c->tile_count.as<int32_t>(), c->tile_off.as<int32_t>(),
                      c->survivors.as<Survivor>(), cap_guess, c->stream);
    HIPCHK(c, hipEventSynchronize(c->ev_sv));
  } else HIPCHK(c, hipStreamSynchronize(c->stream));
  HIPCHK(c, hipGetLastError());
  const int32_t n_sv = sv_off[ng];
  const bool compacted = cap_guess > 0 && n_sv <= cap_guess;
  c->sv_cap_guess = n_sv > 0 ? n_sv + n_sv / 4 + 64 : 0;
  HT("cand:n_sv");
  if (c->phase.dbg.prof) fprintf(stderr, "[cand] %d survivors of the count filters in %lld columns, %d reads\n", n_sv, (long long)c->n_cols, c->bv.n_reads);
  HIPCHK(c, c->survivors.reserve(std::max(n_sv, 1) * sizeof(Survivor)));
  HIPCHK(c, c->hist.reserve(std::max<size_t>(n_sv, 1) * 124 * 4 + 64));
  HIPCHK(c, c->cand_tmp.reserve(std::max<size_t>(n_sv, 1) * sizeof(lcr_candidate)));
  HIPCHK(c, c->keep.reserve(((size_t)std::max(n_sv, 1) * 3 + 2) * 4));
  HIPCHK(c, c->d_cand.reserve(std::max<size_t>(n_sv, 1) * sizeof(lcr_candidate)));
  HIPCHK(c, c->d_cand_off.reserve((ng + 1) * 4));
  int32_t* const d_keep = c->keep.as<int32_t>();
  int32_t* const d_pos = d_keep + std::max(n_sv, 1);
  int32_t* const d_idx = d_pos + std::max(n_sv, 1) + 1;
  c->h_cand.clear();
  c->h_cand_off.assign(ng + 1, 0);
  c->hits_valid = false;
  if (n_sv) {
    const bool tiles_ok = c->dp.ont && p->max_depth <= 65535u;
    const bool hist_tiles = tiles_ok && c->dbg_hist_tiles >= 0 && (c->dbg_hist_tiles > 0 || (int64_t)n_sv * 8 >= c->n_cols);
    if (!compacted) HIPCHK(c, lcr_fill_async(c->hist.p, 0, (size_t)n_sv * 124 * 4 + 64, c->stream));
    c->hits_valid = !hist_tiles && c->dbg_k3_hits != 0;
    c->hits_n_sv = n_sv;
    if (c->hits_valid) {
      HIPCHK(c, c->hit_cnt.reserve(std::max<size_t>(c->bv.n_reads, 1) * 4));
      HIPCHK(c, c->hit_list.reserve(std::max<size_t>(c->bv.n_reads, 1) * LCR_HITS * 8));
      HIPCHK(c, c->ovf_list.reserve(std::max<size_t>(c->bv.n_reads, 1) * 4));
    }
    { Timer t(c, LCR_K_CAND_HIST);
      if (!compacted)
      launch_k2_compact(c->bv, c->dp, c->tile_region.as<int32_t>(), c->tile_col0.as<int32_t>(), nt, c->n_cols,
                        c->planes.as<uint32_t>(), c->flags.as<uint8_t>(), c->tile_count.as<int32_t>(), c->tile_off.as<int32_t>(),
                        c->survivors.as<Survivor>(), n_sv, c->stream);
      if (hist_tiles)
        launch_k2_hist_tiles(c->bv, c->tile_col0.as<int32_t>(), nt, c->tile_count.as<int32_t>(), c->tile_off.as<int32_t>(), c->survivors.as<Survivor>(),
                             c->chunk_off.as<int32_t>(), c->chunks.p, c->k0_items.as<unsigned long long>(), c->hist.as<uint32_t>(), c->stream);
      else
        launch_k2_hist(c->bv, c->dp, c->read_bin.as<ReadBin>(), c->survivors.as<Survivor>(), c->tile_off.as<int32_t>(), nt, n_sv, c->hist.as<uint32_t>(),
                       c->hits_valid ? c->hit_cnt.as<int32_t>() : nullptr, c->hit_list.p, (int32_t*)(c->hist.as<uint32_t>() + (size_t)n_sv * 124), c->ovf_list.as<int32_t>(),
                       c->stream); }
    { Timer t(c, LCR_K_CAND_GT);
      launch_k2_gt(c->dp, c->survivors.as<Survivor>(), n_sv, c->hist.as<uint32_t>(), c->bv.start0,
                   c->cand_tmp.as<lcr_candidate>(), d_keep, c->stream); }
  }
  HIPCHK(c, c->h_stage[1].reserve(std::max<size_t>(n_sv, 1) * sizeof(lcr_candidate)));
  HIPCHK(c, c->h_stage[2].reserve((size_t)(ng + 1) * 4));
  { lcr_candidate* hp = nullptr; int32_t* ho = nullptr;
    HIPCHK(c, hipHostGetDevicePointer((void**)&hp, c->h_stage[1].p, 0));
    HIPCHK(c, hipHostGetDevicePointer((void**)&ho, c->h_stage[2].p, 0));
    if (ng == 0) c->h_stage[2].as<int32_t>()[0] = 0;
    launch_k2_finish(c->scan_tmp, c->cand_tmp.as<lcr_candidate>(), d_keep, n_sv, c->sv_region_off.as<int32_t>(), ng, d_pos, d_idx,
                     c->d_cand.as<lcr_candidate>(), c->d_cand_off.as<int32_t>(), p->dense_win, p->min_dense_cnt, c->stream, hp, ho); }
  HT("cand:finish_q");
  c->cand_dl_other = false;
  HIPCHK(c, c->region_rows.reserve(std::max(ng, 1) * 4));
  HIPCHK(c, c->h_stage[3].reserve(std::max(ng, 1) * 4));
  HIPCHK(c, c->row_region_off.reserve((ng + 1) * 4));
  { int32_t* d_rr = nullptr;
    HIPCHK(c, hipHostGetDevicePointer((void**)&d_rr, c->h_stage[3].p, 0));
    launch_k3_rows_offsets(c->bv, c->d_cand.as<lcr_candidate>(), c->d_cand_off.as<int32_t>(), c->region_rows.as<int32_t>(), c->row_region_off.as<int32_t>(), c->stream, d_rr); }
  if (!c->ev_cand) HIPCHK(c, hipEventCreateWithFlags(&c->ev_cand, hipEventDisableTiming));
  HIPCHK(c, hipEventRecord(c->ev_cand, c->stream));
  HIPCHK(c, hipGetLastError());
  c->cand_pending = true;
  c->have_cand = true;
  HT("cand:ret");
  c->have_frag = c->have_phase = c->cand_used = false;
  return LCR_OK;
}

int lcr_import_candidates(lcr_ctx* c, const lcr_params* p, int32_t mem, int32_t n_sites, const int64_t* pos0, const uint8_t* genotype,
                          const float* qual) {
  HT("import");
  if (!c) return LCR_E_ARG;
  if (!p || n_sites < 0 || (mem != LCR_MEM_HOST && mem != LCR_MEM_DEVICE)) {
    c->err = "lcr_import_candidates: null params, n_sites < 0 or mem not LCR_MEM_HOST / LCR_MEM_DEVICE";
    return LCR_E_ARG;
  }
  if (n_sites > 0 && (!pos0 || !genotype || !qual)) { c->err = "lcr_import_candidates: null site array"; return LCR_E_ARG; }
  if (!c->have_planes) { c->err = "lcr_import_candidates before lcr_pileup"; return LCR_E_STATE; }
  if (mem == LCR_MEM_HOST)
    for (int32_t i = 0; i < n_sites; i++)
      if (genotype[i] > 4 || (i > 0 && pos0[i - 1] >= pos0[i])) {
        c->err = "lcr_import_candidates: sites must be sorted by position without duplicates, genotype codes 0-4 (site " + std::to_string(i) + ")";
        return LCR_E_ARG;
      }
  HIPCHK(c, hipSetDevice(c->device));
  { int rc = phase_settle(c); if (rc) return rc; }
  if (c->cand_pending && c->cand_dl_other) HIPCHK(c, hipEventSynchronize(c->ev_cand_dl));
  const int ng = c->bv.n_regions;
  const int64_t* d_pos = nullptr; const uint8_t* d_gt = nullptr; const float* d_q = nullptr;
  { int rc = upload(c, c->imp_pos, pos0, (size_t)n_sites, &d_pos, mem); if (rc) return rc; }
  { int rc = upload(c, c->imp_gt, genotype, (size_t)n_sites, &d_gt, mem); if (rc) return rc; }
  { int rc = upload(c, c->imp_q, qual, (size_t)n_sites, &d_q, mem); if (rc) return rc; }
  if (mem == LCR_MEM_DEVICE && n_sites > 0) {
    HIPCHK(c, c->h_imp_bad.reserve(64));
    int32_t* bad = c->h_imp_bad.as<int32_t>();
    *bad = 0;
    int32_t* d_bad = nullptr;
    HIPCHK(c, hipHostGetDevicePointer((void**)&d_bad, bad, 0));
    launch_k2_import_check(d_pos, d_gt, n_sites, d_bad, c->stream);
    if (!c->ev_imp) HIPCHK(c, hipEventCreateWithFlags(&c->ev_imp, hipEventDisableTiming));
    HIPCHK(c, hipEventRecord(c->ev_imp, c->stream));
    HIPCHK(c, hipEventSynchronize(c->ev_imp));
    if (*(volatile int32_t*)bad) { c->err = "lcr_import_candidates: sites must be sorted by position without duplicates, genotype codes 0-4"; return LCR_E_ARG; }
  }
  c->res_valid = false;
  HIPCHK(c, c->imp_cnt.reserve(std::max(ng, 1) * 4));
  HIPCHK(c, c->d_cand.reserve(std::max<size_t>(n_sites, 1) * sizeof(lcr_candidate)));
  HIPCHK(c, c->d_cand_off.reserve((ng + 1) * 4));
  HIPCHK(c, c->h_stage[1].reserve(std::max<size_t>(n_sites, 1) * sizeof(lcr_candidate)));
  HIPCHK(c, c->h_stage[2].reserve((size_t)(ng + 1) * 4));
  c->h_cand.clear();
  c->h_cand_off.assign(ng + 1, 0);
  c->hits_valid = false;
  { lcr_candidate* hp = nullptr; int32_t* ho = nullptr;
    HIPCHK(c, hipHostGetDevicePointer((void**)&hp, c->h_stage[1].p, 0));
    HIPCHK(c, hipHostGetDevicePointer((void**)&ho, c->h_stage[2].p, 0));
    if (ng == 0) c->h_stage[2].as<int32_t>()[0] = 0;
    Timer t(c, LCR_K_CAND_IMPORT);
    launch_k2_import_count(c->bv, d_pos, d_gt, d_q, n_sites, c->imp_cnt.as<int32_t>(), c->stream);
    launch_scan_i32(c->scan_tmp, c->imp_cnt.as<int32_t>(), c->d_cand_off.as<int32_t>(), ng, c->d_cand_off.as<int32_t>() + ng, c->stream);
    launch_k2_import_emit(c->bv, c->n_cols, c->planes.as<uint32_t>(), d_pos, d_gt, d_q, n_sites, c->d_cand_off.as<int32_t>(),
                          c->d_cand.as<lcr_candidate>(), c->stream, hp, ho); }
  c->cand_dl_other = false;
  HIPCHK(c, c->region_rows.reserve(std::max(ng, 1) * 4));
  HIPCHK(c, c->h_stage[3].reserve(std::max(ng, 1) * 4));
  HIPCHK(c, c->row_region_off.reserve((ng + 1) * 4));
  { int32_t* d_rr = nullptr;
    HIPCHK(c, hipHostGetDevicePointer((void**)&d_rr, c->h_stage[3].p, 0));
    launch_k3_rows_offsets(c->bv, c->d_cand.as<lcr_candidate>(), c->d_cand_off.as<int32_t>(), c->region_rows.as<int32_t>(), c->row_region_off.as<int32_t>(), c->stream, d_rr); }
  if (!c->ev_cand) HIPCHK(c, hipEventCreateWithFlags(&c->ev_cand, hipEventDisableTiming));
  HIPCHK(c, hipEventRecord(c->ev_cand, c->stream));
  HIPCHK(c, hipGetLastError());
  c->cand_pending = true;
  c->have_cand = true;
  c->have_frag = c->have_phase = c->cand_used = false;
  HT("import:ret");
  return LCR_OK;
}

int lcr_get_candidates(lcr_ctx* c, lcr_candidate_list* out) {
  if (!c || !out) return LCR_E_ARG;
  if (!c->have_cand) { c->err = "lcr_get_candidates before lcr_candidates"; return LCR_E_STATE; }
  { int rc = cand_settle(c); if (rc) return rc; }
  { int rc = phase_settle(c); if (rc) return rc; }
  out->n_cand = (int32_t)c->h_cand.size();
  out->n_regions = c->bv.n_regions;
  out->cand = c->h_cand.data();
  out->region_off = c->h_cand_off.data();
  return LCR_OK;
}

static int cand_settle(lcr_ctx* c) {
  if (!c->cand_pending) return LCR_OK;
  HIPCHK(c, hipEventSynchronize(c->ev_cand));
  if (c->cand_dl_other) HIPCHK(c, hipEventSynchronize(c->ev_cand_dl));
  const int ng = c->bv.n_regions;
  memcpy(c->h_cand_off.data(), c->h_stage[2].p, (size_t)(ng + 1) * 4);
  c->h_cand.assign(c->h_stage[1].as<lcr_candidate>(), c->h_stage[1].as<lcr_candidate>() + c->h_cand_off[ng]);
  c->cand_pending = false;
  return LCR_OK;
}

static int frag_settle(lcr_ctx* c) {
  if (!c->nnz_pending) return LCR_OK;
  HIPCHK(c, hipEventSynchronize(c->ev_nnz));
  c->nnz = c->h_nnz.as<int64_t>()[c->bv.n_regions];
  c->nnz_pending = false;
  return LCR_OK;
}

int lcr_fragments(lcr_ctx* c, const lcr_params* p) {
  HT("frag");
  if (!c || !p) return LCR_E_ARG;
  if (!c->have_cand) { c->err = "lcr_fragments before lcr_candidates"; return LCR_E_STATE; }
  if (c->cand_used) { c->err = "lcr_fragments after lcr_phase: the phase stage has rewritten the candidate records; run the candidate stage again"; return LCR_E_STATE; }
  if (p->min_linkers == 0) { c->err = "min_linkers must be > 0 (fragment.rs:252)"; return LCR_E_ARG; }
  HIPCHK(c, hipSetDevice(c->device));
  const int ng = c->bv.n_regions;
  c->min_linkers = p->min_linkers;
  const int nr_cap = c->bv.n_reads;
  HIPCHK(c, c->row_cnt.reserve(std::max(nr_cap, 1) * 4));
  HIPCHK(c, c->frag_tmp_col.reserve((size_t)std::max(nr_cap, 1) * launch_k3_inline() * 4));
  HIPCHK(c, c->frag_tmp_val.reserve((size_t)std::max(nr_cap, 1) * launch_k3_inline()));
  HIPCHK(c, c->row_links.reserve(std::max(nr_cap, 1) * 4));
  HIPCHK(c, c->row_ptr.reserve((std::max(nr_cap, 1) + 1) * 8));
  if (nr_cap) HIPCHK(c, lcr_fill_async(c->row_cnt.p, 0, (size_t)nr_cap * 4, c->stream));
  HT("frag:memset_q");
  K3Hits hits{};
  if (c->hits_valid) {
    const int32_t* d_keep = c->keep.as<int32_t>();
    hits = K3Hits{c->hit_cnt.as<int32_t>(), c->hit_list.p, (const int32_t*)(c->hist.as<uint32_t>() + (size_t)c->hits_n_sv * 124), c->ovf_list.as<int32_t>(),
                  d_keep, d_keep + std::max(c->hits_n_sv, 1)};
  }
  { Timer t(c, LCR_K_FRAG_COUNT);
    launch_k3_count(c->bv, c->read_bin.as<ReadBin>(), c->d_cand.as<lcr_candidate>(), c->d_cand_off.as<int32_t>(), c->row_region_off.as<int32_t>(), nr_cap,
                    c->row_cnt.as<int32_t>(), c->row_links.as<uint32_t>(), c->frag_tmp_col.as<int32_t>(), c->frag_tmp_val.as<uint8_t>(), hits, c->stream);
    launch_scan_i32_to_i64(c->scan_tmp, c->row_cnt.as<int32_t>(), c->row_ptr.as<int64_t>(), nr_cap, c->stream); }
  HIPCHK(c, c->h_nnz.reserve((size_t)(ng + 1) * 8));
  HIPCHK(c, c->region_e_off.reserve((size_t)(ng + 1) * 8));
  if (!c->ev_nnz) HIPCHK(c, hipEventCreateWithFlags(&c->ev_nnz, hipEventDisableTiming));
  { int64_t* d_nnz = nullptr;
    HIPCHK(c, hipHostGetDevicePointer((void**)&d_nnz, c->h_nnz.p, 0));
    launch_k3_region_entries(c->row_ptr.as<int64_t>(), c->row_region_off.as<int32_t>(), ng, c->region_e_off.as<int64_t>(), c->stream, d_nnz); }
  HIPCHK(c, hipEventRecord(c->ev_nnz, c->stream));
  c->nnz_pending = true;
  HT("frag:count_q");
  { int rc = cand_settle(c); if (rc) return rc; }
  if (c->phase.dbg.prof && c->hits_valid) {
  HT("frag:cand_settled");
    int32_t n_ovf = 0;
    HIPCHK(c, hipMemcpy(&n_ovf, c->hist.as<uint32_t>() + (size_t)c->hits_n_sv * 124, 4, hipMemcpyDeviceToHost));
    fprintf(stderr, "[frag] %d reads with more than %d survivor hits (walked again)\n", n_ovf, LCR_HITS);
  }
  const int32_t* rr = c->h_stage[3].as<int32_t>();
  c->h_row_region_off.assign(ng + 1, 0);
  for (int g = 0; g < ng; g++) c->h_row_region_off[g + 1] = c->h_row_region_off[g] + rr[g];
  c->n_rows = c->h_row_region_off[ng];
  const int nrow = c->n_rows;
  int64_t bound = 0;
  for (int g = 0; g < ng; g++) bound += (int64_t)rr[g] * (c->h_cand_off[g + 1] - c->h_cand_off[g]);
  int64_t cap = bound;
  if (bound > ((int64_t)1 << 28)) {
    int rc = frag_settle(c);
    if (rc) return rc;
    cap = c->nnz;
  }
  HIPCHK(c, c->col.reserve(std::max<int64_t>(cap, 1) * 4));
  HIPCHK(c, c->val.reserve(std::max<int64_t>(cap, 1)));
  { Timer t(c, LCR_K_FRAG_FILL);
    launch_k3_fill(c->bv, c->read_bin.as<ReadBin>(), c->d_cand.as<lcr_candidate>(), c->d_cand_off.as<int32_t>(), c->row_region_off.as<int32_t>(), nrow,
                   c->row_cnt.as<int32_t>(), c->row_ptr.as<int64_t>(), c->frag_tmp_col.as<int32_t>(), c->frag_tmp_val.as<uint8_t>(),
                   c->col.as<int32_t>(), c->val.as<uint8_t>(), hits, c->stream); }
  HIPCHK(c, hipGetLastError());
  c->have_frag = true;
  HT("frag:ret");
  c->have_phase = false;
  return LCR_OK;
}

int lcr_get_candidates_device(lcr_ctx* c, const lcr_candidate** dev_cand, int32_t* n_cand) {
  if (!c || !dev_cand || !n_cand) return LCR_E_ARG;
  if (!c->have_cand) { c->err = "lcr_get_candidates_device before lcr_candidates"; return LCR_E_STATE; }
  { int rc = cand_settle(c); if (rc) return rc; }
  { int rc = phase_settle(c); if (rc) return rc; }
  *dev_cand = c->d_cand.as<lcr_candidate>();
  *n_cand = (int32_t)c->h_cand.size();
  return LCR_OK;
}

int lcr_get_fragmat(lcr_ctx* c, lcr_fragmat* out) {
  if (!c || !out) return LCR_E_ARG;
  if (!c->have_frag) { c->err = "lcr_get_fragmat before lcr_fragments"; return LCR_E_STATE; }
  { int rc = frag_settle(c); if (rc) return rc; }
  const int nrow = c->n_rows, ng = c->bv.n_regions;
  const int64_t nnz = c->nnz;
  HIPCHK(c, c->h_row_ptr.reserve((nrow + 1) * 8));
  HIPCHK(c, c->h_row_read.reserve(std::max(nrow, 1) * 4));
  HIPCHK(c, c->h_col.reserve(std::max<int64_t>(nnz, 1) * 4));
  HIPCHK(c, c->h_val.reserve(std::max<int64_t>(nnz, 1)));
  HIPCHK(c, c->h_row_fp.reserve(std::max(nrow, 1)));
  HIPCHK(c, c->h_row_links.reserve(std::max(nrow, 1) * 4));
  HIPCHK(c, hipMemcpyAsync(c->h_row_ptr.p, c->row_ptr.p, (size_t)(nrow + 1) * 8, hipMemcpyDeviceToHost, c->stream));
  if (nrow) HIPCHK(c, hipMemcpyAsync(c->h_row_links.p, c->row_links.p, (size_t)nrow * 4, hipMemcpyDeviceToHost, c->stream));
  if (nnz) {
    HIPCHK(c, hipMemcpyAsync(c->h_col.p, c->col.p, (size_t)nnz * 4, hipMemcpyDeviceToHost, c->stream));
    HIPCHK(c, hipMemcpyAsync(c->h_val.p, c->val.p, (size_t)nnz, hipMemcpyDeviceToHost, c->stream));
  }
  HIPCHK(c, hipStreamSynchronize(c->stream));
  int32_t* rread = c->h_row_read.as<int32_t>();
  uint8_t* fp = c->h_row_fp.as<uint8_t>();
  const uint32_t* links = c->h_row_links.as<uint32_t>();
  for (int g = 0; g < ng; g++)
    for (int r = c->h_row_region_off[g]; r < c->h_row_region_off[g + 1]; r++) rread[r] = c->h_read_begin[g] + (r - c->h_row_region_off[g]);
  for (int r = 0; r < nrow; r++) fp[r] = links[r] >= c->min_linkers ? 1 : 0;
  out->n_rows = nrow; out->nnz = nnz; out->n_regions = ng;
  out->row_region_off = c->h_row_region_off.data();
  out->row_ptr = c->h_row_ptr.as<int64_t>(); out->row_read = rread; out->col = c->h_col.as<int32_t>();
  out->val = c->h_val.as<uint8_t>(); out->row_for_phasing = fp; out->row_links = links;
  return LCR_OK;
}

int lcr_phase(lcr_ctx* c, const lcr_params* p) {
  if (!c || !p) return LCR_E_ARG;
  if (!c->have_frag) { c->err = "lcr_phase before lcr_fragments"; return LCR_E_STATE; }
  if (c->cand_used) { c->err = "lcr_phase after lcr_phase: the phase stage has rewritten the candidate records; run the candidate stage again"; return LCR_E_STATE; }
  if (p->ld_weight_threshold != 1) { c->err = "ld_weight_threshold must be 1: SNPFrag::phase is only ever called with 1 (thread.rs:166)"; return LCR_E_ARG; }
  HIPCHK(c, hipSetDevice(c->device));
  { int rc = frag_settle(c); if (rc) return rc; }
  PhaseInputs in;
  in.n_regions = c->bv.n_regions; in.n_rows = c->n_rows; in.nnz = c->nnz;
  in.row_region_off = c->h_row_region_off.data(); in.cand_region_off = c->h_cand_off.data();
  in.region_start0 = c->h_start0.data();
  in.region_e_off = c->h_nnz.as<int64_t>();
  in.d_row_ptr = c->row_ptr.as<int64_t>(); in.d_col = c->col.as<int32_t>(); in.d_val = c->val.as<uint8_t>();
  in.d_row_links = c->row_links.as<uint32_t>();
  in.cand = &c->h_cand;
  in.d_cand = c->d_cand.as<lcr_candidate>(); in.d_cand_off = c->d_cand_off.as<int32_t>();
  in.d_row_region_off = c->row_region_off.as<int32_t>(); in.d_start0 = c->bv.start0;
  Timer t(c, LCR_K_PHASE);
  c->cand_used = true;
  int rc = c->phase.run(in, *p, c->stream, &c->err);
  if (rc) {
    if (c->phase.q_first) (void)hipStreamSynchronize(c->phase.q_first);
    if (c->phase.side) (void)hipStreamSynchronize(c->phase.side);
    if (c->phase.aux) (void)hipStreamSynchronize(c->phase.aux);
    return rc;
  }
  c->have_phase = true;
  c->res_valid = true; c->res_ng = c->bv.n_regions;
  c->phase_slot = c->bound_slot >= 0 ? c->bound_slot : (c->bound_host ? -2 : -1);
  return LCR_OK;
}

int lcr_discover_regions(lcr_ctx* c, int32_t mem, int32_t n_reads, const int32_t* ref_start, const int32_t* ref_end,
                         int64_t contig_len, lcr_region_list* out) {
  if (!c || !out || n_reads < 0 || contig_len < 0 || contig_len > 0x7FFFFFF0ll) return LCR_E_ARG;
  HIPCHK(c, hipSetDevice(c->device));
  c->rl_start0.clear(); c->rl_len.clear(); c->rl_max.clear();
  out->n_regions = 0; out->start0 = nullptr; out->len = nullptr; out->max_cov = nullptr;
  if (n_reads == 0 || contig_len == 0) return LCR_OK;
  const int32_t *d_s = ref_start, *d_e = ref_end;
  if (mem == LCR_MEM_HOST) {
    HIPCHK(c, c->rd_start.reserve((size_t)n_reads * 4)); HIPCHK(c, c->rd_end.reserve((size_t)n_reads * 4));
    { int rc2 = upload_bytes(c, c->rd_start.p, ref_start, (size_t)n_reads * 4); if (rc2) return rc2; rc2 = upload_bytes(c, c->rd_end.p, ref_end, (size_t)n_reads * 4); if (rc2) return rc2; }
    d_s = c->rd_start.as<int32_t>(); d_e = c->rd_end.as<int32_t>();
  }
  int64_t w_lo = contig_len, w_hi = 0;
  if (mem == LCR_MEM_HOST) {
    for (int32_t r = 0; r < n_reads; r++) {
      const int64_t s = ref_start[r], e = std::min<int64_t>(ref_end[r], contig_len);
      if (s >= 0 && s < e) { w_lo = std::min(w_lo, s); w_hi = std::max(w_hi, e); }
    }
  } else {
    HIPCHK(c, c->rd_cnt.reserve(16));
    int32_t init[2] = {INT_MAX, 0}, got[2] = {INT_MAX, 0};
    HIPCHK(c, hipMemcpyAsync(c->rd_cnt.p, init, 8, hipMemcpyHostToDevice, c->stream));
    launch_k5_span_window(d_s, d_e, n_reads, contig_len, c->rd_cnt.as<int32_t>(), c->stream);
    HIPCHK(c, hipMemcpyAsync(got, c->rd_cnt.p, 8, hipMemcpyDeviceToHost, c->stream));
    HIPCHK(c, hipStreamSynchronize(c->stream));
    if (got[1] > 0) { w_lo = got[0]; w_hi = got[1]; }
  }
  if (w_hi <= w_lo) return LCR_OK;
  const int64_t full_len = contig_len;
  contig_len = w_hi - w_lo;
  const size_t nd = (size_t)contig_len + 2;
  HIPCHK(c, c->rd_diff.reserve(nd * 4)); HIPCHK(c, c->rd_ex.reserve((nd + 1) * 4));
  HIPCHK(c, hipMemsetAsync(c->rd_diff.p, 0, nd * 4, c->stream));
  launch_k5_span_diff(d_s, d_e, n_reads, full_len, w_lo, c->rd_diff.as<uint32_t>(), c->stream);
  launch_scan_i32(c->scan_tmp, (const int32_t*)c->rd_diff.p, c->rd_ex.as<int32_t>(), (int32_t)nd, nullptr, c->stream);
  const int32_t nb = (int32_t)((contig_len + 1023) / 1024);
  HIPCHK(c, c->rd_cnt.reserve(((size_t)nb + 1) * 4)); HIPCHK(c, c->rd_off.reserve(((size_t)nb + 2) * 4));
  launch_k5_bounds(false, c->rd_ex.as<int32_t>(), contig_len, nb, c->rd_cnt.as<int32_t>(), nullptr, nullptr, nullptr, c->stream);
  launch_scan_i32(c->scan_tmp, c->rd_cnt.as<int32_t>(), c->rd_off.as<int32_t>(), nb, c->rd_off.as<int32_t>() + nb, c->stream);
  int32_t n_isl = 0;
  HIPCHK(c, hipMemcpyAsync(&n_isl, c->rd_off.as<int32_t>() + nb, 4, hipMemcpyDeviceToHost, c->stream));
  HIPCHK(c, hipStreamSynchronize(c->stream));
  HIPCHK(c, hipGetLastError());
  if (n_isl == 0) return LCR_OK;
  HIPCHK(c, c->rd_s.reserve((size_t)n_isl * 4)); HIPCHK(c, c->rd_e.reserve((size_t)n_isl * 4)); HIPCHK(c, c->rd_max.reserve((size_t)n_isl * 4));
  launch_k5_bounds(true, c->rd_ex.as<int32_t>(), contig_len, nb, nullptr, c->rd_off.as<int32_t>(), c->rd_s.as<int32_t>(), c->rd_e.as<int32_t>(), c->stream);
  launch_k5_island_max(c->rd_ex.as<int32_t>(), c->rd_s.as<int32_t>(), c->rd_e.as<int32_t>(), n_isl, c->rd_max.as<uint32_t>(), c->stream);
  std::vector<int32_t> hs(n_isl), he(n_isl);
  std::vector<uint32_t> hm(n_isl);
  HIPCHK(c, hipMemcpyAsync(hs.data(), c->rd_s.p, (size_t)n_isl * 4, hipMemcpyDeviceToHost, c->stream));
  HIPCHK(c, hipMemcpyAsync(he.data(), c->rd_e.p, (size_t)n_isl * 4, hipMemcpyDeviceToHost, c->stream));
  HIPCHK(c, hipMemcpyAsync(hm.data(), c->rd_max.p, (size_t)n_isl * 4, hipMemcpyDeviceToHost, c->stream));
  HIPCHK(c, hipStreamSynchronize(c->stream));
  HIPCHK(c, hipGetLastError());
  uint32_t running = 0;
  int64_t pend = -1;
  for (int i = 0; i < n_isl; i++) {
    hs[i] += (int32_t)w_lo; he[i] += (int32_t)w_lo;
    running = std::max(running, hm[i]);
    if (pend < 0) pend = hs[i];
    if ((int64_t)he[i] > pend) {
      c->rl_start0.push_back(pend); c->rl_len.push_back((int32_t)(he[i] - pend + 1)); c->rl_max.push_back(running);
      pend = -1; running = 0;
    }
  }
  out->n_regions = (int32_t)c->rl_start0.size();
  out->start0 = c->rl_start0.data(); out->len = c->rl_len.data(); out->max_cov = c->rl_max.data();
  return LCR_OK;
}

int lcr_get_phase_result(lcr_ctx* c, lcr_phase_result* out) {
  if (!c || !out) return LCR_E_ARG;
  if (!c->have_phase) { c->err = "lcr_get_phase_result before lcr_phase"; return LCR_E_STATE; }
  { int rc = phase_settle(c); if (rc) return rc; }
  out->n_rows = c->n_rows; out->n_regions = c->bv.n_regions;
  out->haplotag = c->phase.r_haplotag; out->assignment = c->phase.r_assignment;
  out->phase_set = c->phase.r_phase_set; out->objective = c->phase.objective.data();
  return LCR_OK;
}

int lcr_get_read_records_device(lcr_ctx* c, const lcr_read_record** dev_rec, int32_t* n_rows) {
  if (!c || !dev_rec || !n_rows) return LCR_E_ARG;
  if (!c->have_phase) { c->err = "lcr_get_read_records_device before lcr_phase"; return LCR_E_STATE; }
  HIPCHK(c, hipSetDevice(c->device));
  { int rc = phase_settle(c); if (rc) return rc; }
  static_assert(sizeof(lcr_read_record) == 12, "lcr_read_record is 12 bytes");
  { int rc = read_records_fresh(c); if (rc) return rc; }
  *dev_rec = c->phase.d_read_rec.as<lcr_read_record>();
  *n_rows = c->n_rows;
  return LCR_OK;
}

static int read_records_fresh(lcr_ctx* c) {
  if (!c->phase.read_rec_stale) return LCR_OK;
  std::vector<lcr_read_record> h((size_t)std::max(c->n_rows, 0));
  for (int r = 0; r < c->n_rows; r++) h[r] = lcr_read_record{r, c->phase.r_haplotag[r], c->phase.r_assignment[r], 0, c->phase.r_phase_set[r]};
  if (c->n_rows) { const int rc2 = upload_bytes(c, c->phase.d_read_rec.p, h.data(), h.size() * sizeof(lcr_read_record)); if (rc2) return rc2; HIPCHK(c, hipStreamSynchronize(c->stream)); }
  c->phase.read_rec_stale = false;
  return LCR_OK;
}

int lcr_collect_phase(lcr_ctx* c, lcr_phase_collected* out) {
  if (!c || !out) return LCR_E_ARG;
  if (!c->res_valid) { c->err = "lcr_collect_phase: no phase results (call it after lcr_phase and before the next lcr_candidates)"; return LCR_E_STATE; }
  HIPCHK(c, hipSetDevice(c->device));
  { int rc = phase_settle(c); if (rc) return rc; }
  { int rc = read_records_fresh(c); if (rc) return rc; }
  out->n_regions = c->res_ng; out->n_rows = c->n_rows; out->n_cand = (int32_t)c->h_cand.size(); out->pad_ = 0;
  out->cand = c->h_cand.data(); out->cand_region_off = c->h_cand_off.data(); out->row_region_off = c->h_row_region_off.data();
  out->haplotag = c->phase.r_haplotag; out->assignment = c->phase.r_assignment; out->phase_set = c->phase.r_phase_set;
  out->objective = c->phase.objective.data();
  out->dev_cand = c->d_cand.as<lcr_candidate>(); out->dev_read_rec = c->phase.d_read_rec.as<lcr_read_record>();
  return LCR_OK;
}

int lcr_ctx_set_async_phase(lcr_ctx* c, int on) {
  if (!c) return LCR_E_ARG;
  HIPCHK(c, hipSetDevice(c->device));
  { int rc = phase_settle(c); if (rc) return rc; }
  c->phase.dbg.async_phase = on != 0;
  if (on) {
    const char* q = getenv("GPU_MAX_HW_QUEUES");
    if (!q || atoi(q) < 8) {
      c->err = "asynchronous phase stage: GPU_MAX_HW_QUEUES is unset or below 8 in this process's environment -- the HIP runtime then shares hardware queues "
               "between the stage's streams (results are the same, the overlap is lost); export GPU_MAX_HW_QUEUES=8 before the process starts";
      return LCR_W_HW_QUEUES;
    }
  }
  return LCR_OK;
}

int lcr_ctx_set_lock_dir(lcr_ctx* c, const char* dir) {
  if (!c || !dir) return LCR_E_ARG;
  c->phase.lock_dir = dir;
  return LCR_OK;
}

int lcr_debug_set(lcr_ctx* c, const char* key, int64_t value) {
  if (!c || !key) return LCR_E_ARG;
  PhaseDebug& d = c->phase.dbg;
  const std::string k(key);
  if (k == "phase_prof") d.prof = (int)value;
  else if (k == "post_host") d.post_host = (int)value;
  else if (k == "grid_min_entries") d.grid_min = value;
  else if (k == "grid_generic") d.grid_generic = (int)value;
  else if (k == "post_half") d.post_half = (int)value;
  else if (k == "enum_force_big") d.enum_force_big = (int)value;
  else if (k == "enum_force_stream") d.enum_force_stream = (int)value;
  else if (k == "host_threads") d.host_threads = (int)value;
  else if (k == "async_phase") d.async_phase = value != 0;
  else if (k == "host_trace") g_lcr_host_trace = value != 0;
  else if (k == "own_fill") g_lcr_own_fill = value != 0;
  else if (k == "fill_selftest") {
    HIPCHK(c, hipSetDevice(c->device));
    const size_t N = 4096;
    DevBuf buf;
    struct Drain { hipStream_t s; ~Drain() { (void)hipStreamSynchronize(s); } } drain{c->stream};
    HIPCHK(c, buf.reserve(4 * N));
    std::vector<uint8_t> host(4 * N), want(4 * N);
    for (size_t off = 0; off < 18; off++)
      for (size_t len : {(size_t)0, (size_t)1, (size_t)15, (size_t)16, (size_t)17, (size_t)255, (size_t)1000 + off, (size_t)2049}) {
        HIPCHK(c, hipMemsetAsync(buf.p, 0xAB, 4 * N, c->stream));
        std::fill(want.begin(), want.end(), (uint8_t)0xAB);
        uint8_t* base = buf.as<uint8_t>();
        HIPCHK(c, lcr_fill_async(base + off, 0x5C, len, c->stream));
        std::fill(want.begin() + off, want.begin() + off + len, (uint8_t)0x5C);
        void* const ptrs[4] = {base + N + off, base + 2 * N + 3, nullptr, base + 3 * N + off};
        const int vals[4] = {0x80, 0, 7, 0xFF};
        const size_t sizes[4] = {len, 33, 0, len / 2};
        HIPCHK(c, lcr_fill_multi_async(4, ptrs, vals, sizes, c->stream));
        std::fill(want.begin() + N + off, want.begin() + N + off + len, (uint8_t)0x80);
        std::fill(want.begin() + 2 * N + 3, want.begin() + 2 * N + 3 + 33, (uint8_t)0);
        std::fill(want.begin() + 3 * N + off, want.begin() + 3 * N + off + len / 2, (uint8_t)0xFF);
        HIPCHK(c, hipMemcpyAsync(host.data(), buf.p, 4 * N, hipMemcpyDeviceToHost, c->stream));
        HIPCHK(c, hipStreamSynchronize(c->stream));
        if (host != want) { c->err = "fill_selftest: a fill kernel wrote other bytes than asked (offset " + std::to_string(off) + ", length " + std::to_string(len) + ")"; return LCR_E_DEVICE; }
      }
  }
  else if (k == "chain_ties") d.chain_ties = value != 0;
  else if (k == "redo_lds") d.redo_lds = (int)std::max<int64_t>(0, std::min<int64_t>(value, 128 * 1024));
  else if (k == "tie_arith") d.tie_arith = (int)std::max<int64_t>(0, std::min<int64_t>(value, 3));
  else if (k == "timing_mask") c->timing_mask = (uint32_t)value;
  else if (k == "hist_tiles") c->dbg_hist_tiles = value > 0 ? 1 : value < 0 ? -1 : 0;
  else if (k == "k3_hits") c->dbg_k3_hits = value != 0;
  else if (k == "fuse_filter") c->dbg_fuse_filter = value != 0;
  else if (k == "spec_compact") c->dbg_spec_compact = value != 0;
  else if (k == "grid_spec_batch") d.spec_batch = (int)value;
  else if (k == "grid_spec_lanes") d.spec_lanes = (int)std::max<int64_t>(1, std::min<int64_t>(value, 16));
  else { c->err = "lcr_debug_set: unknown key " + k; return LCR_E_ARG; }
  return LCR_OK;
}

int lcr_get_ld_blocks(lcr_ctx* c, int32_t region, int32_t* n_blocks, const int32_t** block_off, const int32_t** snp_idx) {
  if (!c || !n_blocks || !block_off || !snp_idx) return LCR_E_ARG;
  if (!c->have_phase) { c->err = "lcr_get_ld_blocks before lcr_phase"; return LCR_E_STATE; }
  if (region < 0 || region >= c->bv.n_regions) { c->err = "lcr_get_ld_blocks: no such region"; return LCR_E_ARG; }
  { int rc = phase_settle(c); if (rc) return rc; }
  PhaseInputs in;
  in.n_regions = c->bv.n_regions;
  in.cand_region_off = c->h_cand_off.data();
  const int rc = c->phase.ld_blocks(in, region, &c->ld_off, &c->ld_snps, c->stream, &c->err);
  if (rc != LCR_OK) return rc;
  *n_blocks = (int32_t)c->ld_off.size() - 1; *block_off = c->ld_off.data(); *snp_idx = c->ld_snps.data();
  return LCR_OK;
}

int lcr_get_tie_census(lcr_ctx* c, uint64_t out[8]) {
  if (!c || !out) return LCR_E_ARG;
  if (!c->have_phase) { c->err = "lcr_get_tie_census before lcr_phase"; return LCR_E_STATE; }
  { int rc = phase_settle(c); if (rc) return rc; }
  for (int i = 0; i < 8; i++) out[i] = i < TIE_NCTR ? (uint64_t)c->phase.tie_census[i] : 0;
  return LCR_OK;
}

}
```

longcallr_amd/csrc/lcr_dev.h:

```cpp
#pragma once
#include <hip/hip_runtime.h>
#include <climits>
#include <stdint.h>

#include <string>
#include <vector>

#include "../../include/lcr.h"

#ifndef LCR_TILE
#define LCR_TILE 256
#endif
#define LCR_BLOCK 256
#define LCR_WAVE 64

struct BatchView {
  int32_t n_reads, n_regions;
  int64_t n_bases;
  const int32_t* pos;
  const int32_t* seq_len;
  const int32_t* lead;
  const int32_t* trail;
  const uint8_t* flags;
  const uint64_t* seq_off;
  const uint64_t* cig_off;
  const uint32_t* n_cig;
  const uint8_t* bases;
  const uint8_t* quals;
  const uint32_t* cigar;
  const int64_t* start0;
  const int32_t* len;
  const int64_t* col_off;
  const int32_t* read_begin;
  const uint8_t* ref;
  const int32_t* region_first_tile;
  const int32_t* read_region;
  int32_t* error_flag;
  int32_t* read_rend;
};

struct ReadBin {
  int32_t rel_pos;
  int32_t vec;
  int32_t ftile;
  int32_t n_cig;
  int64_t gbase;
  uint64_t seq_off, cig_off;
  int32_t lead, reb;
  int32_t flags, pad_;
  int64_t pad2_;
};
static_assert(sizeof(ReadBin) == 64, "ReadBin must be 64 bytes");

struct DevParams {
  int32_t ont;
  int32_t dist_to_end, polya_len;
  uint32_t min_baseq, min_depth, max_depth, min_qual, low_cnt_cut, min_linkers;
  int32_t use_strand_bias;
  float min_af, min_af_intron, low_frac_cut;
  float sor_threshold;
  int32_t dbg;
};

#define REC_OFF_MASK 0xFFFFFFFFFFull
#define REC_KIND_D 0xFFFFFFFFFFull
#define REC_KIND_I 0xFFFFFFFFFEull
#define REC_KIND_N 0xFFFFFFFFFDull

struct Survivor {
  int64_t gcol;
  int32_t region;
  int32_t col;
  uint8_t ref_base, allele1, allele2, n_alt;
  uint32_t cnt1, cnt2, depth;
  uint32_t ts_fwd, ts_rev;
  float af1, af2;
};

#define HIPCHK(ctx, expr)                                                              \
  do {                                                                                 \
    hipError_t e_ = (expr);                                                            \
    if (e_ != hipSuccess) {                                                            \
      (ctx)->err = std::string(#expr) + ": " + hipGetErrorString(e_);                  \
      return LCR_E_DEVICE;                                                             \
    }                                                                                  \
  } while (0)

void* lcr_cache_take(int host, size_t want, size_t* cap);
bool lcr_cache_put(int host, void* p, size_t cap);

extern int g_lcr_host_trace;
void lcr_host_trace_mark(const char* tag);
void lcr_host_trace_flush();
#define HT(tag) do { if (g_lcr_host_trace) lcr_host_trace_mark(tag); } while (0)

extern int g_lcr_own_fill;
hipError_t lcr_fill_async(void* p, int byte, size_t bytes, hipStream_t s);
hipError_t lcr_fill_multi_async(int n , void* const* ptrs, const int* bytes_val, const size_t* sizes, hipStream_t s);

struct DevBuf {
  void* p = nullptr;
  size_t cap = 0;
  DevBuf() = default;
  DevBuf(const DevBuf&) = delete; DevBuf& operator=(const DevBuf&) = delete;
  ~DevBuf() { if (p && !lcr_cache_put(0, p, cap)) (void)hipFree(p); }
  hipError_t reserve(size_t bytes) {
    if (bytes <= cap) return hipSuccess;
    if (p) { (void)hipDeviceSynchronize(); if (!lcr_cache_put(0, p, cap)) (void)hipFree(p); }
    p = nullptr;
    cap = 0;
    size_t want = bytes + bytes / 8 + 256;
    if ((p = lcr_cache_take(0, want, &cap)) != nullptr) return hipSuccess;
    hipError_t e = hipMalloc(&p, want);
    if (e == hipSuccess) cap = want; else p = nullptr;
    return e;
  }
  template <class T> T* as() const { return reinterpret_cast<T*>(p); }
};
struct HostBuf {
  void* p = nullptr;
  size_t cap = 0;
  HostBuf() = default;
  HostBuf(const HostBuf&) = delete; HostBuf& operator=(const HostBuf&) = delete;
  ~HostBuf() { if (p && !lcr_cache_put(1, p, cap)) (void)hipHostFree(p); }
  hipError_t reserve(size_t bytes) {
    if (bytes <= cap) return hipSuccess;
    if (p) { (void)hipDeviceSynchronize(); if (!lcr_cache_put(1, p, cap)) (void)hipHostFree(p); }
    p = nullptr;
    cap = 0;
    size_t want = bytes + bytes / 8 + 256;
    if ((p = lcr_cache_take(1, want, &cap)) != nullptr) return hipSuccess;
    hipError_t e = hipHostMalloc(&p, want, hipHostMallocDefault);
    if (e == hipSuccess) cap = want; else p = nullptr;
    return e;
  }
  template <class T> T* as() const { return reinterpret_cast<T*>(p); }
};

struct PhaseLutDev {
  int64_t fe[31], f1e[31];
  int64_t f_homref, f_homvar, f_het0, f_log2;
};

void launch_k0_region_setup(const int64_t* start0, const int32_t* len, const int64_t* col_off, const int32_t* read_begin, int32_t ng,
                            int32_t* first_tile, int64_t* h_start0, int32_t* h_len, int64_t* h_col_off, int32_t* h_read_begin,
                            hipStream_t s);
void launch_k0_tiles(const int32_t* first_tile, int32_t n_regions, int32_t* tile_region, int32_t* tile_col0, hipStream_t s);
void launch_k0_read_region(const BatchView& b, int32_t* read_region, hipStream_t s);
void launch_k0_tiles_read_region(const BatchView& b, const int32_t* first_tile, int32_t* tile_region, int32_t* tile_col0, int32_t* read_region, hipStream_t s);
void launch_k0_pack(const BatchView& b, ReadBin* out, int32_t* order_flag , hipStream_t s);
void launch_k0_bind_a(const int64_t* start0, const int32_t* len, const int64_t* col_off, const int32_t* read_begin, int32_t ng,
                      int32_t* first_tile, int64_t* h_start0, int32_t* h_len, int64_t* h_col_off, int32_t* h_read_begin,
                      const uint64_t* cig_off, const uint32_t* n_cig, int32_t nr, int64_t n_cigar, int32_t* out, hipStream_t s);
void launch_k0_bind_b(const BatchView& b, ReadBin* rbin, int32_t* order_flag, int32_t* read_region, int32_t n_tiles, int32_t* tile_region,
                      int32_t* tile_col0, uint64_t cig0, int32_t opb, int32_t n_blocks, int32_t* blk_first_read, hipStream_t s);
void launch_k0_cig_check(const uint64_t* cig_off, const uint32_t* n_cig, int32_t nr, int64_t n_cigar, int32_t* out, hipStream_t s);
void launch_k0_cig_compact(const uint32_t* cigar, const uint64_t* cig_off, const uint32_t* n_cig, const int32_t* new_off, int32_t nr,
                           uint32_t* out, uint64_t* out_off, hipStream_t s);
int launch_k0_opb();
void launch_k0_block_reads(const ReadBin* rbin, int32_t nr, uint64_t cig0, int32_t opb, int32_t n_blocks, int32_t* blk_first_read, hipStream_t s);
void launch_k0_ops(const BatchView& b, const ReadBin* rb, const int32_t* blk_first_read, uint64_t cig0, uint32_t n_ops, int ont, int D,
                   int32_t n_tiles, int32_t* tile_fill, int32_t* tile_nchunks, int32_t* tile_ndiff, void* ctl, unsigned int* acct ,
                   unsigned int pool_sub , unsigned long long* recs, unsigned int desc_sub, uint32_t* desc_tile, void* desc_val ,
                   void* read_scan , hipStream_t s);
int launch_k0_acct_words();
int launch_k0_acct_slots();
void launch_k0_desc_bin(const void* ctl, const unsigned int* acct, unsigned int desc_sub, const uint32_t* desc_tile, const void* desc_val,
                        const int32_t* chunk_off, int32_t* cursor , void* sorted , int32_t n_blocks_hint,
                        hipStream_t s);
size_t launch_k1_tiles_tmp_words(int32_t n_tiles);
void launch_k1_tiles_a(int32_t n_tiles, const int32_t* tile_fill, const int32_t* tile_ndiff, const int32_t* tile_nent, int32_t* tmp ,
                       const unsigned int* acct, int32_t n_acct, unsigned int* ctl, unsigned int* host_ctl , hipStream_t s);
void launch_k1_tiles_b(int32_t n_tiles, const int32_t* tile_fill, const int32_t* tile_ndiff, const int32_t* tile_nent, int32_t* tmp,
                       int32_t* tile_nbase, int32_t* ent_off, int32_t* order, hipStream_t s);
void launch_k1_pileup(const BatchView& b, const DevParams& p, const int32_t* tile_region, const int32_t* tile_col0,
                      int32_t n_tiles, int64_t n_cols, const int32_t* tile_fill, const int32_t* chunk_off, const void* chunks,
                      const unsigned long long* recs, const int32_t* tile_nbase, uint32_t* planes, const int32_t* order,
                      const int32_t* tiles_tmp , hipStream_t s,
                      uint8_t* flt_flags , int32_t* flt_count );
void launch_k1_zonefix(const BatchView& b, const ReadBin* rbin, int D, int L, int64_t n_cols, uint32_t* planes, hipStream_t s);
void launch_k2_filter(const BatchView& b, const DevParams& p, const int32_t* tile_region, const int32_t* tile_col0,
                      int32_t n_tiles, int64_t n_cols, const uint32_t* planes, const int32_t* tile_fill, uint8_t* flags,
                      int32_t* tile_count, hipStream_t s);
void launch_gather_i32(const int32_t* src, const int32_t* idx, int32_t n, int32_t n_src, const int32_t* total, int32_t* out, hipStream_t s,
                       int32_t* host_out = nullptr );
void launch_scan_i32(DevBuf& tmp, const int32_t* in, int32_t* out_excl, int32_t n, int32_t* total, hipStream_t s);
void launch_k2_compact(const BatchView& b, const DevParams& p, const int32_t* tile_region, const int32_t* tile_col0,
                       int32_t n_tiles, int64_t n_cols, const uint32_t* planes, const uint8_t* flags,
                       const int32_t* tile_count, const int32_t* tile_off, Survivor* out, int32_t out_cap, hipStream_t s);
float lcr_device_sor_threshold(hipStream_t s);
#define LCR_HITS 16
void launch_k2_hist(const BatchView& b, const DevParams& p, const ReadBin* rbin, const Survivor* sv, const int32_t* tile_off , int32_t n_tiles, int32_t n_sv,
                    uint32_t* hist , int32_t* hit_cnt , void* hit_list ,
                    int32_t* ovf_cnt , int32_t* ovf_list , hipStream_t s);
void launch_k2_hist_tiles(const BatchView& b, const int32_t* tile_col0, int32_t n_tiles, const int32_t* tile_count,
                          const int32_t* tile_off, const Survivor* sv, const int32_t* ent_off, const void* ents, const unsigned long long* recs,
                          uint32_t* hist, hipStream_t s);
void launch_k2_gt(const DevParams& p, const Survivor* sv, int32_t n_sv, const uint32_t* hist, const int64_t* start0,
                  lcr_candidate* out, int32_t* keep, hipStream_t s);
void launch_k2_finish(DevBuf& scan_tmp, const lcr_candidate* tmp, const int32_t* keep, int32_t n_sv, const int32_t* sv_region_off,
                      int32_t n_regions, int32_t* pos, int32_t* idx, lcr_candidate* out, int32_t* cand_off, uint32_t dense_win,
                      uint32_t min_dense_cnt, hipStream_t s, lcr_candidate* h_cand = nullptr, int32_t* h_off = nullptr);
void launch_k2_import_count(const BatchView& b, const int64_t* pos0, const uint8_t* gt, const float* qual, int32_t n_sites, int32_t* count , hipStream_t s);
void launch_k2_import_emit(const BatchView& b, int64_t n_cols, const uint32_t* planes, const int64_t* pos0, const uint8_t* gt, const float* qual,
                           int32_t n_sites, const int32_t* cand_off , lcr_candidate* out, hipStream_t s,
                           lcr_candidate* h_cand , int32_t* h_off );
void launch_k2_import_check(const int64_t* pos0, const uint8_t* gt, int32_t n_sites, int32_t* bad , hipStream_t s);
void launch_k3_row_offsets(const int32_t* region_rows, int32_t ng, int32_t* row_region_off, hipStream_t s);
void launch_k3_region_entries(const int64_t* row_ptr, const int32_t* row_region_off, int32_t ng, int64_t* region_e_off, hipStream_t s, int64_t* host_out = nullptr);
struct K3Hits {
  const int32_t* hit_cnt; const void* hit_list; const int32_t* ovf_cnt; const int32_t* ovf_list;
  const int32_t* keep; const int32_t* pos;
};
void launch_k3_count(const BatchView& b, const ReadBin* rbin, const lcr_candidate* cand, const int32_t* cand_region_off,
                     const int32_t* row_region_off, int32_t n_rows, int32_t* row_cnt, uint32_t* row_links, int32_t* tmp_col,
                     uint8_t* tmp_val, const K3Hits& hits, hipStream_t s);
void launch_k3_fill(const BatchView& b, const ReadBin* rbin, const lcr_candidate* cand, const int32_t* cand_region_off,
                    const int32_t* row_region_off, int32_t n_rows, int32_t* row_cnt, const int64_t* row_ptr, const int32_t* tmp_col,
                    const uint8_t* tmp_val, int32_t* col, uint8_t* val, const K3Hits& hits, hipStream_t s);
int launch_k3_inline();
void launch_k3_rows(const BatchView& b, const lcr_candidate* cand, const int32_t* cand_region_off, int32_t* region_rows,
                    hipStream_t s, int32_t* host_out = nullptr );
void launch_k3_rows_offsets(const BatchView& b, const lcr_candidate* cand, const int32_t* cand_region_off, int32_t* region_rows, int32_t* row_region_off,
                            hipStream_t s, int32_t* host_rows = nullptr);
void launch_scan_i32_to_i64(DevBuf& tmp, const int32_t* in, int64_t* out_excl, int32_t n, hipStream_t s);

void launch_k5_span_window(const int32_t* ref_start, const int32_t* ref_end, int32_t n, int64_t contig_len, int32_t* out , hipStream_t s);
void launch_k5_span_diff(const int32_t* ref_start, const int32_t* ref_end, int32_t n, int64_t contig_len, int64_t lo , uint32_t* diff, hipStream_t s);
void launch_k5_bounds(bool write, const int32_t* ex, int64_t contig_len, int32_t n_blocks, int32_t* blk_cnt, const int32_t* blk_off,
                      int32_t* starts, int32_t* ends, hipStream_t s);
void launch_k5_island_max(const int32_t* ex, const int32_t* starts, const int32_t* ends, int32_t n_islands, uint32_t* maxcov, hipStream_t s);

#ifdef __HIPCC__
__device__ __forceinline__ int base_code(uint8_t b) {
  switch (b) {
    case 'A': case 'a': return 0;
    case 'C': case 'c': return 1;
    case 'G': case 'g': return 2;
    case 'T': case 't': return 3;
    default: return -1;
  }
}
__device__ __forceinline__ int iabs_(int x) { return x < 0 ? -x : x; }

__device__ __forceinline__ bool in_end_zone(int c, int lead, int reb, int D) {
  return iabs_(c - lead) < D || iabs_(c - reb) < D;
}

__device__ __forceinline__ bool polya_masked(const uint8_t* __restrict__ seq, int seq_len, int c, int L, uint8_t R) {
  int lo = c - L;
  int hi = c + L;
  if (lo < 0) lo = 0;
  if (hi > seq_len - 1) hi = seq_len - 1;
  if (hi - lo + 1 < L) return false;
  int run = 1;
  uint8_t prev = seq[lo];
  bool masked = false;
  for (int i = lo + 1; i <= hi; i++) {
    uint8_t cur = seq[i];
    run = (cur == prev) ? run + 1 : 1;
    prev = cur;
    if (run >= L) {
      int t = i - L + 1;
      if (t >= c - L && t <= c + 1 && cur != R && (cur == 'A' || cur == 'C' || cur == 'G' || cur == 'T')) masked = true;
    }
  }
  return masked;
}


__device__ __forceinline__ int wave_incl_scan(int v) {
  v += __builtin_amdgcn_update_dpp(0, v, 0x111, 0xf, 0xf, false);
  v += __builtin_amdgcn_update_dpp(0, v, 0x112, 0xf, 0xf, false);
  v += __builtin_amdgcn_update_dpp(0, v, 0x114, 0xf, 0xf, false);
  v += __builtin_amdgcn_update_dpp(0, v, 0x118, 0xf, 0xf, false);
  v += __builtin_amdgcn_update_dpp(0, v, 0x142, 0xa, 0xf, false);
  v += __builtin_amdgcn_update_dpp(0, v, 0x143, 0xc, 0xf, false);
  return v;
}

__device__ __forceinline__ int row16_incl_scan(int v) {
  v += __builtin_amdgcn_update_dpp(0, v, 0x111, 0xf, 0xf, false);
  v += __builtin_amdgcn_update_dpp(0, v, 0x112, 0xf, 0xf, false);
  v += __builtin_amdgcn_update_dpp(0, v, 0x114, 0xf, 0xf, false);
  v += __builtin_amdgcn_update_dpp(0, v, 0x118, 0xf, 0xf, false);
  return v;
}

template <class ColFn>
__device__ __forceinline__ void row16_find_sites(bool live, const ReadBin& h, int rend, int s_lo, int s_hi, ColFn site_col, int* cur_out, int* s_end_out) {
  const int lane = threadIdx.x & 63, l16 = lane & 15, rbase = lane & 48;
  int cur = s_hi, s_end = s_hi;
  if (live) {
    const int key = h.rel_pos > 0 ? h.rel_pos : 0;
    bool found_cur = false;
    for (int base = s_lo; base < s_hi; base += 16) {
      const int i = base + l16;
      const int colv = i < s_hi ? site_col(i) : INT_MAX;
      const unsigned int ge_key = (unsigned int)(__ballot(colv >= key) >> rbase) & 0xffffu;
      const unsigned int ge_end = (unsigned int)(__ballot(colv >= rend) >> rbase) & 0xffffu;
      if (!found_cur && ge_key) { cur = base + __ffs((int)ge_key) - 1; found_cur = true; }
      if (ge_end) { s_end = base + __ffs((int)ge_end) - 1; break; }
    }
    if (!found_cur) cur = s_end;
  }
  *cur_out = cur; *s_end_out = s_end;
}

template <class ColFn, class Sink>
__device__ __forceinline__ void row16_walk_range(const BatchView& b, const ReadBin& h, int cur, int s_end, const uint32_t* pre, ColFn site_col, Sink sink) {
  const int lane = threadIdx.x & 63, l16 = lane & 15, rbase = lane & 48;
  if (cur >= s_end) return;
  const uint32_t ncig = (uint32_t)h.n_cig;
  const uint32_t* __restrict__ cg = b.cigar + h.cig_off;
  for (int first = cur; first < s_end; first += 16) {
    const int n = min(16, s_end - first);
    const int my_cc = l16 < n ? site_col(first + l16) : INT_MAX;
    const int last_cc = __shfl(my_cc, rbase + n - 1, 64);
    int myc = -1;
    int ref_cur = h.rel_pos;
    int q_cur = h.lead > 0 ? h.lead : 0;
    int j = 0;
    int cc = __shfl(my_cc, rbase, 64);
    for (uint32_t c0 = 0; c0 < ncig && j < n; c0 += 64) {
      uint32_t w4[4];
      if (pre && c0 == 0) {
#pragma unroll
        for (int k = 0; k < 4; k++) w4[k] = pre[k];
      } else {
#pragma unroll
        for (int k = 0; k < 4; k++) w4[k] = c0 + 16 * k + l16 < ncig ? cg[c0 + 16 * k + l16] : 0u;
      }
#pragma unroll
      for (int k = 0; k < 4; k++) {
        const uint32_t w = w4[k];
        const int op = w & 15, len = (int)(w >> 4);
        const bool is_m = op == 0 || op == 7 || op == 8;
        const int dr = (is_m || op == 2 || op == 3) ? len : 0;
        const int dq = (is_m || op == 1) ? len : 0;
        const int ir = row16_incl_scan(dr), iq = row16_incl_scan(dq);
        const int rs = ref_cur + ir - dr, qs = q_cur + iq - dq;
        const int chunk_end = ref_cur + __shfl(ir, rbase + 15, 64);
        while (j < n && cc < chunk_end) {
          const unsigned int m = (unsigned int)(__ballot(is_m && cc >= rs && cc < rs + len) >> rbase) & 0xffffu;
          if (m) {
            const int L = rbase + __ffs((int)m) - 1;
            const int c = __shfl(qs, L, 64) + (cc - __shfl(rs, L, 64));
            if (l16 == j) myc = c;
          }
          j++;
          cc = __shfl(my_cc, rbase + (j < n ? j : 0), 64);
        }
        ref_cur = chunk_end;
        q_cur += __shfl(iq, rbase + 15, 64);
      }
      if (ref_cur > last_cc) break;
    }
    sink(first + l16, myc, myc >= 0);
  }
}

template <class ColFn, class Sink>
__device__ __forceinline__ void row16_walk_sites(const BatchView& b, bool live, const ReadBin& h, int rend, int s_lo, int s_hi,
                                                 ColFn site_col, Sink sink) {
  int cur, s_end;
  row16_find_sites(live, h, rend, s_lo, s_hi, site_col, &cur, &s_end);
  row16_walk_range(b, h, cur, s_end, nullptr, site_col, sink);
}

#define region_of_read(b_, r_) ((b_).read_region[(r_)])
#endif
```

Before: 5.997 billion.

## Fuse scan chains into single-pass decoupled-lookback kernels and fold gathers, scatter, row offsets

Adds a single-pass scan kernel that uses decoupled lookback with ticketed block ordering and an optional epilogue gather. This replaces the two-kernel scan plus separate gather launches. The k2 scatter and per-region row counting and offsets are folded into k2_dense, using a last-block-done pattern, and several memsets are merged into one multi-fill. The goal is fewer kernel launches and fewer dependent stream steps. In exchange it relies on atomic spinning across blocks and on persistent state that must be reset correctly between calls.

```diff
diff --git a/longcallr_amd/csrc/k2_candidates.hip b/longcallr_amd/csrc/k2_candidates.hip
--- a/longcallr_amd/csrc/k2_candidates.hip
+++ b/longcallr_amd/csrc/k2_candidates.hip
@@ -103,10 +103,106 @@
 }
 __global__ void write_total_i64(const long long* total, int64_t* dst) { *dst = (int64_t)*total; }
 
-void launch_scan_i32(DevBuf& tmp, const int32_t* in, int32_t* out_excl, int32_t n, int32_t* total, hipStream_t s) {
+struct ScanState {
+  unsigned int ticket, done, aux, pad;
+  unsigned long long word[SCAN_FUSED_BLOCKS];
+};
+#define SCAN_STATE_BYTES sizeof(ScanState)
+template <typename OutT>
+struct ScanGather { const int32_t* idx; int32_t n; OutT* out; OutT* host_out; };
+#define LCR_AT_LOAD(p) __hip_atomic_load((p), __ATOMIC_RELAXED, __HIP_MEMORY_SCOPE_AGENT)
+#define LCR_AT_STORE(p, v) __hip_atomic_store((p), (v), __ATOMIC_RELAXED, __HIP_MEMORY_SCOPE_AGENT)
+#define LCR_AT_ADD(p, v) __hip_atomic_fetch_add((p), (v), __ATOMIC_RELAXED, __HIP_MEMORY_SCOPE_AGENT)
+
+template <typename OutT>
+__global__ void __launch_bounds__(LCR_BLOCK) scan_fused(const int32_t* __restrict__ in, OutT* __restrict__ out, int32_t n, ScanState* __restrict__ st, int32_t n_blocks,
+                                                        int32_t* __restrict__ total32, int64_t* __restrict__ total64, ScanGather<OutT> ep) {
+  __shared__ long long wsum[LCR_BLOCK / 64], psum[LCR_BLOCK / 64];
+  __shared__ unsigned int t_s, last_s;
+  const int tid = threadIdx.x, lane = tid & 63, w = tid >> 6;
+  if (tid == 0) t_s = LCR_AT_ADD(&st->ticket, 1u);
+  __syncthreads();
+  const int t = (int)t_s;
+  const long long base = (long long)t * SCAN_TILE + (long long)tid * SCAN_ITEMS;
+  long long v[SCAN_ITEMS], s = 0;
+#pragma unroll
+  for (int k = 0; k < SCAN_ITEMS; k++) { v[k] = (base + k < n) ? (long long)in[base + k] : 0; s += v[k]; }
+  const long long incl = wave_incl_scan_ll(s, lane);
+  if (lane == 63) wsum[w] = incl;
+  __syncthreads();
+  long long add_w = 0;
+  for (int i = 0; i < w; i++) add_w += wsum[i];
+  const long long bsum = wsum[0] + wsum[1] + wsum[2] + wsum[3];
+  if (tid == 0) LCR_AT_STORE(&st->word[t], ((unsigned long long)bsum << 2) | (t == 0 ? 2ull : 1ull));
+  if (w == 0) {
+    long long excl = 0;
+    for (int j = t - 1; j >= 0; j -= 64) {
+      const int at = j - lane;
+      unsigned long long x = 2ull;
+      if (at >= 0) while (((x = LCR_AT_LOAD(&st->word[at])) & 3ull) == 0ull) __builtin_amdgcn_s_sleep(1);
+      const unsigned long long m = __ballot((x & 3ull) == 2ull);
+      const int first = m ? __ffsll((long long)m) - 1 : 64;
+      long long val = lane <= first ? ((long long)x >> 2) : 0;
+      for (int d = 32; d >= 1; d >>= 1) val += __shfl_xor(val, d, 64);
+      excl += val;
+      if (m) break;
+    }
+    if (lane == 0) {
+      if (t > 0) LCR_AT_STORE(&st->word[t], ((unsigned long long)(excl + bsum) << 2) | 2ull);
+      psum[0] = excl;
+    }
+  }
+  __syncthreads();
+  const long long add = psum[0];
+  long long run = incl - s + add_w + add;
+#pragma unroll
+  for (int k = 0; k < SCAN_ITEMS; k++) { if (base + k < n) out[base + k] = (OutT)run; run += v[k]; }
+  if (t == n_blocks - 1 && tid == LCR_BLOCK - 1) {
+    if (total32) *total32 = (int32_t)(add + incl + add_w);
+    if (total64) *total64 = (int64_t)(add + incl + add_w);
+  }
+  if (ep.n > 0) {
+    __syncthreads();
+    const long long lo = (long long)t * SCAN_TILE, hi = lo + SCAN_TILE;
+    const long long tot = add + bsum;
+    static_assert(LCR_BLOCK / 64 == 4, "four waves per scan workgroup");
+    for (int i = tid; i < ep.n; i += LCR_BLOCK) {
+      const int32_t at = ep.idx[i];
+      const bool mine = at < n ? (at >= lo && at < hi) : t == n_blocks - 1;
+      if (!mine) continue;
+      const OutT x = at < n ? out[at] : (OutT)tot;
+      ep.out[i] = x;
+      if (ep.host_out) ep.host_out[i] = x;
+    }
+  }
+  __syncthreads();
+  if (tid == 0) {
+    asm volatile("s_waitcnt vmcnt(0)" ::: "memory");
+    last_s = LCR_AT_ADD(&st->done, 1u) == (unsigned int)(n_blocks - 1);
+  }
+  __syncthreads();
+  if (!last_s) return;
+  for (int j = tid; j < n_blocks; j += LCR_BLOCK) LCR_AT_STORE(&st->word[j], 0ull);
+  if (tid == 0) { LCR_AT_STORE(&st->ticket, 0u); LCR_AT_STORE(&st->done, 0u); }
+}
+
+static long long* scan_tmp_reserve(DevBuf& tmp, int nb, hipStream_t s) {
+  const size_t was = tmp.cap;
+  if (tmp.reserve(SCAN_STATE_BYTES + ((size_t)nb + 2) * sizeof(long long)) != hipSuccess) return nullptr;
+  if (tmp.cap != was) (void)hipMemsetAsync(tmp.p, 0, SCAN_STATE_BYTES, s);
+  return reinterpret_cast<long long*>((char*)tmp.p + SCAN_STATE_BYTES);
+}
+
+void launch_scan_i32(DevBuf& tmp, const int32_t* in, int32_t* out_excl, int32_t n, int32_t* total, hipStream_t s, int fused,
+                     const int32_t* g_idx, int32_t n_gather, int32_t* g_out, int32_t* g_host) {
   const int nb = (n + SCAN_TILE - 1) / SCAN_TILE;
-  (void)tmp.reserve(((size_t)nb + 2) * sizeof(long long));
-  long long* bs = tmp.as<long long>();
+  long long* bs = scan_tmp_reserve(tmp, nb, s);
+  if (!bs) return;
+  if (fused && n > 0 && nb <= SCAN_FUSED_BLOCKS && (n_gather == 0 || total)) {
+    hipLaunchKernelGGL(scan_fused<int32_t>, dim3(nb), dim3(LCR_BLOCK), 0, s, in, out_excl, n, tmp.as<ScanState>(), nb, total, (int64_t*)nullptr,
+                       ScanGather<int32_t>{g_idx, n_gather, g_out, g_host});
+    return;
+  }
   if (n > 0 && nb <= SCAN_FUSED_BLOCKS) {
     hipLaunchKernelGGL(scan_phase1<int32_t>, dim3(nb), dim3(LCR_BLOCK), 0, s, in, out_excl, n, bs);
     hipLaunchKernelGGL(scan_phase3x<int32_t>, dim3(nb), dim3(LCR_BLOCK), 0, s, out_excl, n, bs, nb, total, (int64_t*)nullptr);
@@ -118,11 +214,18 @@
   } else if (total) {
     (void)hipMemsetAsync(total, 0, sizeof(int32_t), s);
   }
-}
-void launch_scan_i32_to_i64(DevBuf& tmp, const int32_t* in, int64_t* out_excl, int32_t n, hipStream_t s) {
+  if (n_gather > 0) launch_gather_i32(out_excl, g_idx, n_gather, n, total, g_out, s, g_host);
+}
+bool launch_scan_i32_to_i64(DevBuf& tmp, const int32_t* in, int64_t* out_excl, int32_t n, hipStream_t s, int fused,
+                            const int32_t* g_idx, int32_t n_gather, int64_t* g_out, int64_t* g_host) {
   const int nb = (n + SCAN_TILE - 1) / SCAN_TILE;
-  (void)tmp.reserve(((size_t)nb + 2) * sizeof(long long));
-  long long* bs = tmp.as<long long>();
+  long long* bs = scan_tmp_reserve(tmp, nb, s);
+  if (!bs) return false;
+  if (fused && n > 0 && nb <= SCAN_FUSED_BLOCKS) {
+    hipLaunchKernelGGL(scan_fused<int64_t>, dim3(nb), dim3(LCR_BLOCK), 0, s, in, out_excl, n, tmp.as<ScanState>(), nb, (int32_t*)nullptr, out_excl + n,
+                       ScanGather<int64_t>{g_idx, n_gather, g_out, g_host});
+    return n_gather > 0;
+  }
   if (n > 0 && nb <= SCAN_FUSED_BLOCKS) {
     hipLaunchKernelGGL(scan_phase1<int64_t>, dim3(nb), dim3(LCR_BLOCK), 0, s, in, out_excl, n, bs);
     hipLaunchKernelGGL(scan_phase3x<int64_t>, dim3(nb), dim3(LCR_BLOCK), 0, s, out_excl, n, bs, nb, (int32_t*)nullptr, out_excl + n);
@@ -134,6 +237,7 @@
   } else {
     (void)hipMemsetAsync(out_excl, 0, sizeof(int64_t), s);
   }
+  return false;
 }
 
 __global__ void k2_sor_threshold(float* out) { *out = strand_odds_ratio(5, 5, 9, 1); }
@@ -496,6 +600,11 @@
   return h;
 }
 
+#define K2_REGION_SCATTER_MAX 1024
+struct K2Region {
+  const lcr_candidate* tmp; const int32_t* keep; const int32_t* pos; const int32_t* sv_region_off;
+  BatchView b; int32_t* region_rows; int32_t* row_region_off; int32_t* host_rows; unsigned int* ticket; unsigned long long* rows_word;
+};
 __global__ void __launch_bounds__(LCR_BLOCK)
 k2_scatter(const lcr_candidate* __restrict__ tmp, const int32_t* __restrict__ keep, const int32_t* __restrict__ pos, int32_t n_sv,
            lcr_candidate* __restrict__ out, const int32_t* __restrict__ sv_region_off, int32_t n_regions, int32_t* __restrict__ cand_off) {
@@ -507,11 +616,19 @@
 }
 __global__ void __launch_bounds__(256)
 k2_dense(lcr_candidate* __restrict__ cand, const int32_t* __restrict__ cand_off, int32_t n_regions, int32_t* __restrict__ idx,
-         uint32_t dense_win, uint32_t min_dense_cnt, lcr_candidate* __restrict__ h_cand, int32_t* __restrict__ h_off) {
+         uint32_t dense_win, uint32_t min_dense_cnt, lcr_candidate* __restrict__ h_cand, int32_t* __restrict__ h_off, K2Region fz) {
   __shared__ int wcnt[4], base_s;
   const int g = blockIdx.x, tid = threadIdx.x, lane = tid & 63, w = tid >> 6;
   const int lo = cand_off[g], hi = cand_off[g + 1];
   int32_t* concat = idx + lo;
+  if (fz.tmp) {
+    const int64_t e0 = (int64_t)fz.sv_region_off[g] * 8, e1 = (int64_t)fz.sv_region_off[g + 1] * 8;
+#pragma unroll 4
+    for (int64_t e = e0 + tid; e < e1; e += 256) {
+      const int s = (int)(e >> 3), wd = (int)(e & 7);
+      if (fz.keep[s]) reinterpret_cast<uint4*>(cand + fz.pos[s])[wd] = reinterpret_cast<const uint4*>(fz.tmp + s)[wd];
+    }
+  }
   if (tid == 0) base_s = 0;
   __syncthreads();
   for (int i0 = lo; i0 < hi; i0 += 256) {
@@ -542,24 +659,88 @@
     sweep(i, (int64_t)dense_win, min_dense_cnt);
     sweep(i, 4, 3u);
   }
-  if (!h_cand) return;
-  __syncthreads();
-  const uint4* src = reinterpret_cast<const uint4*>(cand + lo);
-  uint4* dst = reinterpret_cast<uint4*>(h_cand + lo);
-  const int n16 = (hi - lo) * (int)(sizeof(lcr_candidate) / 16);
-  for (int i = tid; i < n16; i += 256) dst[i] = src[i];
-  if (tid == 0) { h_off[g] = lo; if (g == n_regions - 1) h_off[n_regions] = hi; }
+  if (h_cand) {
+    __syncthreads();
+    const uint4* src = reinterpret_cast<const uint4*>(cand + lo);
+    uint4* dst = reinterpret_cast<uint4*>(h_cand + lo);
+    const int n16 = (hi - lo) * (int)(sizeof(lcr_candidate) / 16);
+    for (int i = tid; i < n16; i += 256) dst[i] = src[i];
+    if (tid == 0) { h_off[g] = lo; if (g == n_regions - 1) h_off[n_regions] = hi; }
+  }
+  if (!fz.region_rows) return;
+  __shared__ unsigned int last_s;
+  __shared__ int rsum[4];
+  if (tid == 0) {
+    int rows = 0;
+    if (hi > lo) {
+      const int64_t last = cand[hi - 1].pos;
+      int a = fz.b.read_begin[g], z = fz.b.read_begin[g + 1];
+      const int rb = a;
+      while (a < z) { const int mid = (a + z) >> 1; if ((int64_t)fz.b.pos[mid] > last) z = mid; else a = mid + 1; }
+      rows = a - rb;
+    }
+    fz.region_rows[g] = rows;
+    if (fz.host_rows) fz.host_rows[g] = rows;
+    LCR_AT_STORE(&fz.rows_word[g], ((unsigned long long)(unsigned int)rows << 1) | 1ull);
+    asm volatile("s_waitcnt vmcnt(0)" ::: "memory");
+    last_s = LCR_AT_ADD(fz.ticket, 1u) == (unsigned int)(n_regions - 1);
+  }
+  __syncthreads();
+  if (!last_s) return;
+  int before = 0;
+  if (tid == 0) fz.row_region_off[0] = 0;
+  for (int g0 = 0; g0 < n_regions; g0 += 256) {
+    const int gg = g0 + tid;
+    int rows = 0;
+    if (gg < n_regions) {
+      unsigned long long x;
+      while ((x = LCR_AT_LOAD(&fz.rows_word[gg])) == 0ull) __builtin_amdgcn_s_sleep(1);
+      rows = (int)(x >> 1);
+      LCR_AT_STORE(&fz.rows_word[gg], 0ull);
+    }
+    const int incl = wave_incl_scan_i(rows, lane);
+    if (lane == 63) rsum[w] = incl;
+    __syncthreads();
+    int mine = before;
+    for (int k = 0; k < w; k++) mine += rsum[k];
+    if (gg < n_regions) fz.row_region_off[gg + 1] = mine + incl;
+    before += rsum[0] + rsum[1] + rsum[2] + rsum[3];
+    __syncthreads();
+  }
+  if (tid == 0) LCR_AT_STORE(fz.ticket, 0u);
+}
+static unsigned long long* region_words_reserve(DevBuf& buf, int n, hipStream_t s) {
+  const size_t was = buf.cap;
+  if (buf.reserve((size_t)std::max(n, 1) * 8) != hipSuccess) return nullptr;
+  if (buf.cap != was) (void)hipMemsetAsync(buf.p, 0, buf.cap, s);
+  return buf.as<unsigned long long>();
 }
 void launch_k2_finish(DevBuf& scan_tmp, const lcr_candidate* tmp, const int32_t* keep, int32_t n_sv, const int32_t* sv_region_off,
                       int32_t n_regions, int32_t* pos , int32_t* idx , lcr_candidate* out,
                       int32_t* cand_off , uint32_t dense_win, uint32_t min_dense_cnt, hipStream_t s,
-                      lcr_candidate* h_cand , int32_t* h_off ) {
+                      lcr_candidate* h_cand , int32_t* h_off ,
+                      const K2Rows* rows ,
+                      int32_t max_region_sv ) {
   static_assert(sizeof(lcr_candidate) % 16 == 0, "k2_dense exports 16-byte words");
-  launch_scan_i32(scan_tmp, keep, pos, n_sv, pos + n_sv, s);
+  if (rows && n_sv > 0 && n_regions > 0) {
+    launch_scan_i32(scan_tmp, keep, pos, n_sv, pos + n_sv, s, 1, sv_region_off, n_regions + 1, cand_off, nullptr);
+    const bool own_scatter = max_region_sv > K2_REGION_SCATTER_MAX;
+    if (own_scatter)
+      hipLaunchKernelGGL(k2_scatter, dim3((unsigned)(((int64_t)n_sv * 8 + LCR_BLOCK - 1) / LCR_BLOCK)), dim3(LCR_BLOCK), 0, s, tmp, keep, pos, n_sv, out,
+                         sv_region_off, -1, cand_off);
+    unsigned long long* const rw = region_words_reserve(*rows->words, n_regions, s);
+    if (!rw) return;
+    ScanState* st = scan_tmp.as<ScanState>();
+    K2Region fz{own_scatter ? nullptr : tmp, keep, pos, sv_region_off, *rows->b, rows->region_rows, rows->row_region_off, rows->host_rows, &st->aux, rw};
+    hipLaunchKernelGGL(k2_dense, dim3(n_regions), dim3(256), 0, s, out, cand_off, n_regions, idx, dense_win, min_dense_cnt, h_cand, h_off, fz);
+    return;
+  }
+  launch_scan_i32(scan_tmp, keep, pos, n_sv, pos + n_sv, s, rows != nullptr);
   if (n_sv > 0) {
     const int64_t nthreads = std::max<int64_t>((int64_t)n_sv * 8, (int64_t)n_regions + 1);
     hipLaunchKernelGGL(k2_scatter, dim3((unsigned)((nthreads + LCR_BLOCK - 1) / LCR_BLOCK)), dim3(LCR_BLOCK), 0, s, tmp, keep, pos, n_sv, out,
                        sv_region_off, n_regions, cand_off);
   } else launch_gather_i32(pos, sv_region_off, n_regions + 1, n_sv, pos + n_sv, cand_off, s);
-  if (n_regions > 0) hipLaunchKernelGGL(k2_dense, dim3(n_regions), dim3(256), 0, s, out, cand_off, n_regions, idx, dense_win, min_dense_cnt, h_cand, h_off);
-}
+  if (n_regions > 0) hipLaunchKernelGGL(k2_dense, dim3(n_regions), dim3(256), 0, s, out, cand_off, n_regions, idx, dense_win, min_dense_cnt, h_cand, h_off, K2Region{});
+  if (rows) launch_k3_rows_offsets(*rows->b, out, cand_off, rows->region_rows, rows->row_region_off, s, rows->host_rows);
+}
diff --git a/longcallr_amd/csrc/lcr_api.hip b/longcallr_amd/csrc/lcr_api.hip
--- a/longcallr_amd/csrc/lcr_api.hip
+++ b/longcallr_amd/csrc/lcr_api.hip
@@ -28,6 +28,7 @@
   bool cand_dl_other = false;
   int bound_slot = -1;
   bool bound_host = false;
+  DevBuf region_words;
   DevBuf scan_tmp, read_region, read_bin, read_rend, tile_region, tile_col0, first_tile, k0_tile_fill, k0_items, tile_nbase, tile_order;
   DevBuf desc_tile, desc_val, chunks, chunk_off;
   DevBuf blk_first_read, read_scan, cig_compact, cig_off_new, cig_new_off32;
@@ -62,6 +63,9 @@
   bool flt_fused = false;
   DevParams flt_dp{};
   int dbg_k3_hits = 1;
+  int dbg_fused_chains = 1;
+  void* pre_hist_p = nullptr; size_t pre_hist_bytes = 0;
+  void* pre_rowcnt_p = nullptr; size_t pre_rowcnt_bytes = 0;
   std::vector<lcr_candidate> h_cand;
   std::vector<int32_t> h_cand_off;
   DevBuf d_cand, d_cand_off;
@@ -608,6 +612,8 @@
   c->dp = to_dev(p, c->sor_thr);
   c->dp.dbg = 0;
   HIPCHK(c, c->planes.reserve(std::max<size_t>((size_t)c->n_cols * LCR_NPLANES, 1) * 4));
+  bool first_fill = true;
+  c->pre_hist_bytes = c->pre_rowcnt_bytes = 0;
   bool gated = false;
   BatchView& b = c->bv;
   const int nt = c->n_tiles;
@@ -639,7 +645,19 @@
     HIPCHK(c, c->desc_tile.reserve(desc_sub64 * nsh * 4));
     HIPCHK(c, c->desc_val.reserve(desc_sub64 * nsh * 8));
     HIPCHK(c, c->chunks.reserve((pool_sub64 * nsh / 16 + desc_sub64 * nsh + 16) * 8));
-    HIPCHK(c, lcr_fill_async(fill, 0, fill_words * 4, c->stream));
+    if (first_fill && c->dbg_fused_chains) {
+      const size_t hist_bytes = (c->dbg_spec_compact && nt > 0 && c->sv_cap_guess > 0) ? (size_t)c->sv_cap_guess * 124 * 4 + 64 : 0;
+      const size_t rc_bytes = (size_t)b.n_reads * 4;
+      if (hist_bytes) HIPCHK(c, c->hist.reserve(hist_bytes));
+      if (rc_bytes) HIPCHK(c, c->row_cnt.reserve(rc_bytes));
+      void* const fp[3] = {fill, c->hist.p, c->row_cnt.p};
+      const int fv[3] = {0, 0, 0};
+      const size_t fs[3] = {fill_words * 4, hist_bytes, rc_bytes};
+      HIPCHK(c, lcr_fill_multi_async(3, fp, fv, fs, c->stream));
+      c->pre_hist_p = c->hist.p; c->pre_hist_bytes = hist_bytes;
+      c->pre_rowcnt_p = c->row_cnt.p; c->pre_rowcnt_bytes = rc_bytes;
+    } else HIPCHK(c, lcr_fill_async(fill, 0, fill_words * 4, c->stream));
+    first_fill = false;
     if (!gated) { HIPCHK(c, c->phase.gate_stream(c->stream)); gated = true; }
     { Timer t(c, LCR_K_SPANS);
       launch_k0_ops(b, c->read_bin.as<ReadBin>(), c->blk_first_read.as<int32_t>(), c->cig0, c->n_ops, c->dp.ont, c->dp.dist_to_end, nt,
@@ -735,15 +753,17 @@
   int32_t* const sv_off = c->h_stage[0].as<int32_t>();
   { int32_t* d_sv = nullptr;
     HIPCHK(c, hipHostGetDevicePointer((void**)&d_sv, sv_off, 0));
-    launch_scan_i32(c->scan_tmp, c->tile_count.as<int32_t>(), c->tile_off.as<int32_t>(), nt, c->total.as<int32_t>(), c->stream);
-    launch_gather_i32(c->tile_off.as<int32_t>(), c->first_tile.as<int32_t>(), ng + 1, nt, c->total.as<int32_t>(), c->sv_region_off.as<int32_t>(), c->stream, d_sv); }
+    launch_scan_i32(c->scan_tmp, c->tile_count.as<int32_t>(), c->tile_off.as<int32_t>(), nt, c->total.as<int32_t>(), c->stream, c->dbg_fused_chains,
+                    c->first_tile.as<int32_t>(), ng + 1, c->sv_region_off.as<int32_t>(), d_sv); }
   const int32_t cap_guess = (c->dbg_spec_compact && nt > 0) ? c->sv_cap_guess : 0;
   if (cap_guess > 0) {
     if (!c->ev_sv) HIPCHK(c, hipEventCreateWithFlags(&c->ev_sv, hipEventDisableTiming));
     HIPCHK(c, hipEventRecord(c->ev_sv, c->stream));
     HIPCHK(c, c->survivors.reserve((size_t)cap_guess * sizeof(Survivor)));
     HIPCHK(c, c->hist.reserve((size_t)cap_guess * 124 * 4 + 64));
-    HIPCHK(c, lcr_fill_async(c->hist.p, 0, (size_t)cap_guess * 124 * 4 + 64, c->stream));
+    const bool pre = c->dbg_fused_chains && c->pre_hist_p == c->hist.p && c->pre_hist_bytes >= (size_t)cap_guess * 124 * 4 + 64;
+    c->pre_hist_bytes = 0;
+    if (!pre) HIPCHK(c, lcr_fill_async(c->hist.p, 0, (size_t)cap_guess * 124 * 4 + 64, c->stream));
     launch_k2_compact(c->bv, c->dp, c->tile_region.as<int32_t>(), c->tile_col0.as<int32_t>(), nt, c->n_cols,
                       c->planes.as<uint32_t>(), c->flags.as<uint8_t>(), c->tile_count.as<int32_t>(), c->tile_off.as<int32_t>(),
                       c->survivors.as<Survivor>(), cap_guess, c->stream);
@@ -751,6 +771,7 @@
   } else HIPCHK(c, hipStreamSynchronize(c->stream));
   HIPCHK(c, hipGetLastError());
   const int32_t n_sv = sv_off[ng];
+  c->pre_hist_bytes = 0;
   const bool compacted = cap_guess > 0 && n_sv <= cap_guess;
   c->sv_cap_guess = n_sv > 0 ? n_sv + n_sv / 4 + 64 : 0;
   HT("cand:n_sv");
@@ -800,16 +821,21 @@
     HIPCHK(c, hipHostGetDevicePointer((void**)&hp, c->h_stage[1].p, 0));
     HIPCHK(c, hipHostGetDevicePointer((void**)&ho, c->h_stage[2].p, 0));
     if (ng == 0) c->h_stage[2].as<int32_t>()[0] = 0;
+    HIPCHK(c, c->region_rows.reserve(std::max(ng, 1) * 4));
+    HIPCHK(c, c->h_stage[3].reserve(std::max(ng, 1) * 4));
+    HIPCHK(c, c->row_region_off.reserve((ng + 1) * 4));
+    int32_t* d_rr = nullptr;
+    HIPCHK(c, hipHostGetDevicePointer((void**)&d_rr, c->h_stage[3].p, 0));
+    const K2Rows rows{&c->bv, c->region_rows.as<int32_t>(), c->row_region_off.as<int32_t>(), d_rr, &c->region_words};
+    int32_t max_region_sv = 0;
+    for (int g = 0; g < ng; g++) max_region_sv = std::max(max_region_sv, sv_off[g + 1] - sv_off[g]);
     launch_k2_finish(c->scan_tmp, c->cand_tmp.as<lcr_candidate>(), d_keep, n_sv, c->sv_region_off.as<int32_t>(), ng, d_pos, d_idx,
-                     c->d_cand.as<lcr_candidate>(), c->d_cand_off.as<int32_t>(), p->dense_win, p->min_dense_cnt, c->stream, hp, ho); }
-  HT("cand:finish_q");
+                     c->d_cand.as<lcr_candidate>(), c->d_cand_off.as<int32_t>(), p->dense_win, p->min_dense_cnt, c->stream, hp, ho,
+                     c->dbg_fused_chains ? &rows : nullptr, max_region_sv);
+    HT("cand:finish_q");
+    if (!c->dbg_fused_chains)
+      launch_k3_rows_offsets(c->bv, c->d_cand.as<lcr_candidate>(), c->d_cand_off.as<int32_t>(), c->region_rows.as<int32_t>(), c->row_region_off.as<int32_t>(), c->stream, d_rr); }
   c->cand_dl_other = false;
-  HIPCHK(c, c->region_rows.reserve(std::max(ng, 1) * 4));
-  HIPCHK(c, c->h_stage[3].reserve(std::max(ng, 1) * 4));
-  HIPCHK(c, c->row_region_off.reserve((ng + 1) * 4));
-  { int32_t* d_rr = nullptr;
-    HIPCHK(c, hipHostGetDevicePointer((void**)&d_rr, c->h_stage[3].p, 0));
-    launch_k3_rows_offsets(c->bv, c->d_cand.as<lcr_candidate>(), c->d_cand_off.as<int32_t>(), c->region_rows.as<int32_t>(), c->row_region_off.as<int32_t>(), c->stream, d_rr); }
   if (!c->ev_cand) HIPCHK(c, hipEventCreateWithFlags(&c->ev_cand, hipEventDisableTiming));
   HIPCHK(c, hipEventRecord(c->ev_cand, c->stream));
   HIPCHK(c, hipGetLastError());
@@ -871,7 +897,7 @@
     if (ng == 0) c->h_stage[2].as<int32_t>()[0] = 0;
     Timer t(c, LCR_K_CAND_IMPORT);
     launch_k2_import_count(c->bv, d_pos, d_gt, d_q, n_sites, c->imp_cnt.as<int32_t>(), c->stream);
-    launch_scan_i32(c->scan_tmp, c->imp_cnt.as<int32_t>(), c->d_cand_off.as<int32_t>(), ng, c->d_cand_off.as<int32_t>() + ng, c->stream);
+    launch_scan_i32(c->scan_tmp, c->imp_cnt.as<int32_t>(), c->d_cand_off.as<int32_t>(), ng, c->d_cand_off.as<int32_t>() + ng, c->stream, c->dbg_fused_chains);
     launch_k2_import_emit(c->bv, c->n_cols, c->planes.as<uint32_t>(), d_pos, d_gt, d_q, n_sites, c->d_cand_off.as<int32_t>(),
                           c->d_cand.as<lcr_candidate>(), c->stream, hp, ho); }
   c->cand_dl_other = false;
@@ -937,7 +963,10 @@
   HIPCHK(c, c->frag_tmp_val.reserve((size_t)std::max(nr_cap, 1) * launch_k3_inline()));
   HIPCHK(c, c->row_links.reserve(std::max(nr_cap, 1) * 4));
   HIPCHK(c, c->row_ptr.reserve((std::max(nr_cap, 1) + 1) * 8));
-  if (nr_cap) HIPCHK(c, lcr_fill_async(c->row_cnt.p, 0, (size_t)nr_cap * 4, c->stream));
+  {
+    const bool pre = c->dbg_fused_chains && c->pre_rowcnt_p == c->row_cnt.p && c->pre_rowcnt_bytes >= (size_t)nr_cap * 4;
+    c->pre_rowcnt_bytes = 0;
+    if (nr_cap && !pre) HIPCHK(c, lcr_fill_async(c->row_cnt.p, 0, (size_t)nr_cap * 4, c->stream)); }
   HT("frag:memset_q");
   K3Hits hits{};
   if (c->hits_valid) {
@@ -945,16 +974,18 @@
     hits = K3Hits{c->hit_cnt.as<int32_t>(), c->hit_list.p, (const int32_t*)(c->hist.as<uint32_t>() + (size_t)c->hits_n_sv * 124), c->ovf_list.as<int32_t>(),
                   d_keep, d_keep + std::max(c->hits_n_sv, 1)};
   }
+  HIPCHK(c, c->h_nnz.reserve((size_t)(ng + 1) * 8));
+  HIPCHK(c, c->region_e_off.reserve((size_t)(ng + 1) * 8));
+  if (!c->ev_nnz) HIPCHK(c, hipEventCreateWithFlags(&c->ev_nnz, hipEventDisableTiming));
+  int64_t* d_nnz = nullptr;
+  HIPCHK(c, hipHostGetDevicePointer((void**)&d_nnz, c->h_nnz.p, 0));
+  bool gathered;
   { Timer t(c, LCR_K_FRAG_COUNT);
     launch_k3_count(c->bv, c->read_bin.as<ReadBin>(), c->d_cand.as<lcr_candidate>(), c->d_cand_off.as<int32_t>(), c->row_region_off.as<int32_t>(), nr_cap,
                     c->row_cnt.as<int32_t>(), c->row_links.as<uint32_t>(), c->frag_tmp_col.as<int32_t>(), c->frag_tmp_val.as<uint8_t>(), hits, c->stream);
-    launch_scan_i32_to_i64(c->scan_tmp, c->row_cnt.as<int32_t>(), c->row_ptr.as<int64_t>(), nr_cap, c->stream); }
-  HIPCHK(c, c->h_nnz.reserve((size_t)(ng + 1) * 8));
-  HIPCHK(c, c->region_e_off.reserve((size_t)(ng + 1) * 8));
-  if (!c->ev_nnz) HIPCHK(c, hipEventCreateWithFlags(&c->ev_nnz, hipEventDisableTiming));
-  { int64_t* d_nnz = nullptr;
-    HIPCHK(c, hipHostGetDevicePointer((void**)&d_nnz, c->h_nnz.p, 0));
-    launch_k3_region_entries(c->row_ptr.as<int64_t>(), c->row_region_off.as<int32_t>(), ng, c->region_e_off.as<int64_t>(), c->stream, d_nnz); }
+    gathered = launch_scan_i32_to_i64(c->scan_tmp, c->row_cnt.as<int32_t>(), c->row_ptr.as<int64_t>(), nr_cap, c->stream, c->dbg_fused_chains,
+                                      c->row_region_off.as<int32_t>(), ng + 1, c->region_e_off.as<int64_t>(), d_nnz); }
+  if (!gathered) launch_k3_region_entries(c->row_ptr.as<int64_t>(), c->row_region_off.as<int32_t>(), ng, c->region_e_off.as<int64_t>(), c->stream, d_nnz);
   HIPCHK(c, hipEventRecord(c->ev_nnz, c->stream));
   c->nnz_pending = true;
   HT("frag:count_q");
@@ -1250,6 +1281,7 @@
   else if (k == "timing_mask") c->timing_mask = (uint32_t)value;
   else if (k == "hist_tiles") c->dbg_hist_tiles = value > 0 ? 1 : value < 0 ? -1 : 0;
   else if (k == "k3_hits") c->dbg_k3_hits = value != 0;
+  else if (k == "fused_chains") c->dbg_fused_chains = value != 0;
   else if (k == "fuse_filter") c->dbg_fuse_filter = value != 0;
   else if (k == "spec_compact") c->dbg_spec_compact = value != 0;
   else if (k == "grid_spec_batch") d.spec_batch = (int)value;
diff --git a/longcallr_amd/csrc/lcr_dev.h b/longcallr_amd/csrc/lcr_dev.h
--- a/longcallr_amd/csrc/lcr_dev.h
+++ b/longcallr_amd/csrc/lcr_dev.h
@@ -184,7 +184,8 @@
                       int32_t* tile_count, hipStream_t s);
 void launch_gather_i32(const int32_t* src, const int32_t* idx, int32_t n, int32_t n_src, const int32_t* total, int32_t* out, hipStream_t s,
                        int32_t* host_out = nullptr );
-void launch_scan_i32(DevBuf& tmp, const int32_t* in, int32_t* out_excl, int32_t n, int32_t* total, hipStream_t s);
+void launch_scan_i32(DevBuf& tmp, const int32_t* in, int32_t* out_excl, int32_t n, int32_t* total, hipStream_t s, int fused = 0,
+                     const int32_t* g_idx = nullptr, int32_t n_gather = 0, int32_t* g_out = nullptr, int32_t* g_host = nullptr);
 void launch_k2_compact(const BatchView& b, const DevParams& p, const int32_t* tile_region, const int32_t* tile_col0,
                        int32_t n_tiles, int64_t n_cols, const uint32_t* planes, const uint8_t* flags,
                        const int32_t* tile_count, const int32_t* tile_off, Survivor* out, int32_t out_cap, hipStream_t s);
@@ -198,9 +199,11 @@
                           uint32_t* hist, hipStream_t s);
 void launch_k2_gt(const DevParams& p, const Survivor* sv, int32_t n_sv, const uint32_t* hist, const int64_t* start0,
                   lcr_candidate* out, int32_t* keep, hipStream_t s);
+struct K2Rows { const BatchView* b; int32_t* region_rows; int32_t* row_region_off; int32_t* host_rows; DevBuf* words; };
 void launch_k2_finish(DevBuf& scan_tmp, const lcr_candidate* tmp, const int32_t* keep, int32_t n_sv, const int32_t* sv_region_off,
                       int32_t n_regions, int32_t* pos, int32_t* idx, lcr_candidate* out, int32_t* cand_off, uint32_t dense_win,
-                      uint32_t min_dense_cnt, hipStream_t s, lcr_candidate* h_cand = nullptr, int32_t* h_off = nullptr);
+                      uint32_t min_dense_cnt, hipStream_t s, lcr_candidate* h_cand = nullptr, int32_t* h_off = nullptr,
+                      const K2Rows* rows = nullptr, int32_t max_region_sv = 0);
 void launch_k2_import_count(const BatchView& b, const int64_t* pos0, const uint8_t* gt, const float* qual, int32_t n_sites, int32_t* count , hipStream_t s);
 void launch_k2_import_emit(const BatchView& b, int64_t n_cols, const uint32_t* planes, const int64_t* pos0, const uint8_t* gt, const float* qual,
                            int32_t n_sites, const int32_t* cand_off , lcr_candidate* out, hipStream_t s,
@@ -223,7 +226,8 @@
                     hipStream_t s, int32_t* host_out = nullptr );
 void launch_k3_rows_offsets(const BatchView& b, const lcr_candidate* cand, const int32_t* cand_region_off, int32_t* region_rows, int32_t* row_region_off,
                             hipStream_t s, int32_t* host_rows = nullptr);
-void launch_scan_i32_to_i64(DevBuf& tmp, const int32_t* in, int64_t* out_excl, int32_t n, hipStream_t s);
+bool launch_scan_i32_to_i64(DevBuf& tmp, const int32_t* in, int64_t* out_excl, int32_t n, hipStream_t s, int fused = 0,
+                            const int32_t* g_idx = nullptr, int32_t n_gather = 0, int64_t* g_out = nullptr, int64_t* g_host = nullptr);
 
 void launch_k5_span_window(const int32_t* ref_start, const int32_t* ref_end, int32_t n, int64_t contig_len, int32_t* out , hipStream_t s);
 void launch_k5_span_diff(const int32_t* ref_start, const int32_t* ref_end, int32_t n, int64_t contig_len, int64_t lo , uint32_t* diff, hipStream_t s);
```

Result: no change. 6.054 billion (median of 6 runs) (+1.0%).
